# arkiven4/glow-tts

Hardware: AMD Instinct MI355X
Metric: mel_frames_per_sec_train_step (higher is better)
Workload: dtype bf16; 1 GPU; configs/base.json, LJSpeech-shaped synthetic batches, B=32/GPU, T_x<=150, T_y<=800, bf16 GEMMs; batch_per_gpu=32, T_x=150, T_y=800, batches_rotated=8, padded_frames_per_gpu_step=25600, rows_layout=ragged, graphs_captured=6, parallelism=dp1 (utterance-sharded, RCCL gradient all-reduce, fp32 on the wire), launch=one HIP graph per step (one per ragged-row bucket, captured up front)

## Files before the change

### glow-tts_amd/csrc/wn_boundary.hip

```cpp
#include "common.h"
#include "internal.h"
#include "mfma_frag.h"
#include "../../include/glowtts_hip.h"

namespace {

constexpr int H = 192, C = 160, HALF = 80, NL = 4, G = C / 4;
constexpr int BM = 64;
constexpr int AP = H + 8;
constexpr int XP = 136;
constexpr int ZP = C + 4;
constexpr int RD = 8;
#ifndef WNB_PHASES
#define WNB_PHASES 0
#endif
#if WNB_PHASES
__device__ unsigned long long g_wnb_ph[1024 * 48];
#define PH(i) do { if (threadIdx.x == 0 && blockIdx.x < 1024) g_wnb_ph[blockIdx.x * 48 + (i)] = __builtin_amdgcn_s_memtime(); } while (0)
#else
#define PH(i) do { } while (0)
#endif

template <int NB, int KK>
struct WRing { uint4 v[(KK < RD ? KK : RD)][NB]; };

template <int NB, int KK>
__device__ __forceinline__ void gemm_prefetch(const bf16_t* __restrict__ W, int KS, int nb0, int lane, WRing<NB, KK>& ring)
{
  constexpr int D = KK < RD ? KK : RD;
#pragma unroll
  for (int p = 0; p < D; ++p)
#pragma unroll
    for (int bn = 0; bn < NB; ++bn) ring.v[p][bn] = ldfrag(W, (nb0 + bn) * KS + p, lane);
}
template <int NB, int KK>
__device__ __forceinline__ void gemm_run(const bf16_t* __restrict__ W, int KS, int nb0, const bf16_t* Brow, int lane, WRing<NB, KK>& ring,
                                         f32x16_t (&acc)[NB])
{
  constexpr int D = KK < RD ? KK : RD, CH = 4;
#pragma unroll
  for (int k0 = 0; k0 < KK; k0 += CH) {
#pragma unroll
    for (int kk = k0; kk < k0 + CH && kk < KK; ++kk) {
      const bf16x8_t bfm = *reinterpret_cast<const bf16x8_t*>(Brow + kk * 16);
#pragma unroll
      for (int bn = 0; bn < NB; ++bn) acc[bn] = __builtin_amdgcn_mfma_f32_32x32x16_bf16(asfrag(ring.v[kk % D][bn]), bfm, acc[bn], 0, 0, 0);
    }
    if (k0 + D < KK) {
      __builtin_amdgcn_sched_barrier(0);
#pragma unroll
      for (int kk = k0; kk < k0 + CH && kk + D < KK; ++kk)
#pragma unroll
        for (int bn = 0; bn < NB; ++bn) ring.v[kk % D][bn] = ldfrag(W, (nb0 + bn) * KS + kk + D, lane);
      __builtin_amdgcn_sched_barrier(0);
    }
  }
}

__device__ __forceinline__ void utt_atomic_add(float* __restrict__ dst, float s, int utt, int lane)
{
#pragma unroll
  for (int off = 1; off < 64; off <<= 1) {
    const float v = __shfl_up(s, off);
    const int u = __shfl_up(utt, off);
    if (lane >= off && u == utt) s += v;
  }
  const int un = __shfl_down(utt, 1);
  if ((lane == 63 || un != utt) && s != 0.0f) atomicAdd(dst + utt, s);
}

template <int L>
__device__ __forceinline__ void skip_slice(const u32x4_t (&xr)[6], bf16_t* As, const bf16_t* __restrict__ Wskip, int wm, int wn, int r, int h,
                                           int lane, uint4 (&ring)[RD][3], f32x16_t (&acc)[3])
{
  constexpr int KK = NL * H / 16, kbase = L * (H / 16);
#pragma unroll
  for (int i = 0; i < 6; ++i) {
    const int chunk = threadIdx.x + 256 * i, row = chunk / 24, c8 = chunk - row * 24;
    *reinterpret_cast<u32x4_t*>(As + (L * BM + row) * AP + c8 * 8) = xr[i];
  }
  __syncthreads();
  const bf16_t* brow = As + (L * BM + 32 * wm + r) * AP + 8 * h;
  constexpr int CH = 4;
#pragma unroll
  for (int k0 = 0; k0 < H / 16; k0 += CH) {
#pragma unroll
    for (int k2 = k0; k2 < k0 + CH; ++k2) {
      const bf16x8_t bfm = *reinterpret_cast<const bf16x8_t*>(brow + k2 * 16);
#pragma unroll
      for (int bn = 0; bn < 3; ++bn) acc[bn] = __builtin_amdgcn_mfma_f32_32x32x16_bf16(asfrag(ring[(kbase + k2) % RD][bn]), bfm, acc[bn], 0, 0, 0);
    }
    if (kbase + k0 + RD < KK) {
      __builtin_amdgcn_sched_barrier(0);
#pragma unroll
      for (int k2 = k0; k2 < k0 + CH; ++k2)
#pragma unroll
        for (int bn = 0; bn < 3; ++bn)
          if (kbase + k2 + RD < KK) ring[(kbase + k2) % RD][bn] = ldfrag(Wskip, (3 * wn + bn) * KK + kbase + k2 + RD, lane);
      __builtin_amdgcn_sched_barrier(0);
    }
  }
}

__device__ __forceinline__ float4 sq_gather4(const float* __restrict__ y, int b, int t, int c, int T)
{
  const int p = c >= HALF, cc = c - HALF * p;
  const float* src = y + ((size_t)b * HALF + cc) * T + 2 * t + p;
  return make_float4(src[0], src[(size_t)T], src[2 * (size_t)T], src[3 * (size_t)T]);
}
__device__ __forceinline__ void sq_scatter4(float* __restrict__ y, int b, int t, int c, int T, const float4& v)
{
  const int p = c >= HALF, cc = c - HALF * p;
  float* dst = y + ((size_t)b * HALF + cc) * T + 2 * t + p;
  dst[0] = v.x; dst[(size_t)T] = v.y; dst[2 * (size_t)T] = v.z; dst[3 * (size_t)T] = v.w;
}

__device__ __forceinline__ void coop_store_rows(bf16_t* __restrict__ dst, int ld, const bf16_t* __restrict__ tile, int m0, int R)
{
  constexpr int CPR = H / 8;
#pragma unroll
  for (int i = 0; i < BM * CPR / 256; ++i) {
    const int idx = threadIdx.x + 256 * i, row = idx / CPR, c8 = idx - row * CPR, gm = m0 + row;
    if (gm < R) *reinterpret_cast<uint4*>(dst + (size_t)gm * ld + c8 * 8) = *reinterpret_cast<const uint4*>(tile + row * AP + c8 * 8);
  }
}

constexpr int PF_WGS = 64;
__device__ __forceinline__ void prefetch_images(const void* const (&ptr)[16], const uint32_t (&bytes)[16], int wg, uint32_t* sink)
{
  uint32_t acc = 0;
  const int gid = wg * 256 + threadIdx.x, nthr = PF_WGS * 256;
#pragma unroll
  for (int i = 0; i < 16; ++i) {
    if (!ptr[i]) break;
    const uint4* src = static_cast<const uint4*>(ptr[i]);
    const int n16 = (int)(bytes[i] >> 4);
    for (int c = gid; c < n16; c += 4 * nthr) {
      const uint4 v0 = src[c];
      const uint4 v1 = c + nthr < n16 ? src[c + nthr] : make_uint4(0, 0, 0, 0);
      const uint4 v2 = c + 2 * nthr < n16 ? src[c + 2 * nthr] : make_uint4(0, 0, 0, 0);
      const uint4 v3 = c + 3 * nthr < n16 ? src[c + 3 * nthr] : make_uint4(0, 0, 0, 0);
      acc ^= v0.x ^ v1.y ^ v2.z ^ v3.w;
    }
  }
  if (acc == 0x9E3779B9u && sink) *sink = acc;
}

constexpr int F_AS = 0;
constexpr int F_O = BM * AP * 2;
constexpr int F_Z = F_O + BM * ZP * 4;
constexpr int F_RS = (F_Z + BM * ZP * 4 > NL * BM * AP * 2 ? F_Z + BM * ZP * 4 : NL * BM * AP * 2);
constexpr int F_BIAS = F_RS + BM * 4;
constexpr int FWD_LDS = F_BIAS + 3 * H * 4 + BM * 4;
static_assert(F_O + BM * ZP * 4 <= 3 * BM * AP * 2, "the m | logs tile must stay clear of acts slice 3");

template <bool TAIL, bool HEAD>
__global__ __launch_bounds__(256) void gt_wn_boundary_fwd_kernel(gt_boundary_fwd_args a)
{
  extern __shared__ __attribute__((aligned(16))) unsigned char smem[];
  const int n_tiles = (a.R + BM - 1) / BM;
  if ((int)blockIdx.x >= n_tiles) { prefetch_images(a.pf_ptr, a.pf_bytes, blockIdx.x - n_tiles, reinterpret_cast<uint32_t*>(a.logdet)); return; }
  const int lane = threadIdx.x & 63, wave = threadIdx.x >> 6;
  const int r = lane & 31, h = lane >> 5, wm = wave >> 1, wn = wave & 1;
  const int m0 = blockIdx.x * BM, R = a.R;
  bf16_t* As = reinterpret_cast<bf16_t*>(smem + F_AS);
  float* Ot = reinterpret_cast<float*>(smem + F_O);
  float* Zt = reinterpret_cast<float*>(smem + F_Z);
  float* rowsum = reinterpret_cast<float*>(smem + F_RS);
  const int mrow = m0 + 32 * wm + r;
  const float rm_l = mrow < R ? a.rowmask[mrow] : 0.0f;
  float* Bs = reinterpret_cast<float*>(smem + F_BIAS);
  if (threadIdx.x < 3 * H / 4) {
    const int which = threadIdx.x / (H / 4), o = threadIdx.x - which * (H / 4);
    float4 v = make_float4(0.f, 0.f, 0.f, 0.f);
    if (which == 0) { if (TAIL) v = reinterpret_cast<const float4*>(a.b_skip)[o]; }
    else if (which == 1) { if (TAIL && o < C / 4) v = reinterpret_cast<const float4*>(a.b_end)[o]; }
    else if (HEAD) v = reinterpret_cast<const float4*>(a.b_start)[o];
    reinterpret_cast<float4*>(Bs)[threadIdx.x] = v;
  }
  float* Rm = Bs + 3 * H;
  if (threadIdx.x >= 192) {
    const int row = threadIdx.x - 192;
    Rm[row] = m0 + row < R ? a.rowmask[m0 + row] : 0.0f;
  }
  PH(0);

  if (TAIL) {
    const bf16_t* acts = static_cast<const bf16_t*>(a.acts);
    const bf16_t* Wskip = static_cast<const bf16_t*>(a.w_skip);
    u32x4_t xr[NL][6];
#pragma unroll
    for (int l = 0; l < NL; ++l)
#pragma unroll
      for (int i = 0; i < 6; ++i) {
        const int chunk = threadIdx.x + 256 * i, row = chunk / 24, c8 = chunk - row * 24;
        const int gm = m0 + row < R ? m0 + row : R - 1;
        xr[l][i] = *reinterpret_cast<const u32x4_t*>(acts + (size_t)gm * a.ldacts + l * H + c8 * 8);
      }
    if (threadIdx.x < BM) rowsum[threadIdx.x] = 0.0f;
    f32x16_t acc[3];
    acc_zero<3>(acc);
    constexpr int KK = NL * H / 16;
    uint4 ring[RD][3];
#pragma unroll
    for (int p = 0; p < RD; ++p)
#pragma unroll
      for (int bn = 0; bn < 3; ++bn) ring[p][bn] = ldfrag(Wskip, (3 * wn + bn) * KK + p, lane);
    PH(1);
    skip_slice<0>(xr[0], As, Wskip, wm, wn, r, h, lane, ring, acc);
    skip_slice<1>(xr[1], As, Wskip, wm, wn, r, h, lane, ring, acc);
    skip_slice<2>(xr[2], As, Wskip, wm, wn, r, h, lane, ring, acc);
    skip_slice<3>(xr[3], As, Wskip, wm, wn, r, h, lane, ring, acc);
    PH(2);
    WRing<3, H / 16> ring2;
    gemm_prefetch<3, H / 16>(static_cast<const bf16_t*>(a.w_end), a.ks_end, 3 * wn, lane, ring2);
    bf16_t* wn_out = static_cast<bf16_t*>(a.wn_out);
#pragma unroll
    for (int bn = 0; bn < 3; ++bn)
#pragma unroll
      for (int g = 0; g < 4; ++g) {
        const int n = 32 * (3 * wn + bn) + 8 * g + 4 * h;
        const float4 b4 = *reinterpret_cast<const float4*>(Bs + n);
        const uint2 v = pack4((acc[bn][4 * g] + b4.x) * rm_l, (acc[bn][4 * g + 1] + b4.y) * rm_l,
                              (acc[bn][4 * g + 2] + b4.z) * rm_l, (acc[bn][4 * g + 3] + b4.w) * rm_l);
        *reinterpret_cast<uint2*>(As + (32 * wm + r) * AP + n) = v;
      }
    __syncthreads();
    PH(3);
    coop_store_rows(wn_out, H, As, m0, R);
    float4 cy0[5], cy1[5];
    float crm[5];
#pragma unroll
    for (int k = 0; k < 5; ++k) {
      const int item = threadIdx.x + 256 * k, row = item / 20, c = 4 * (item - row * 20), gm = m0 + row < R ? m0 + row : R - 1;
      cy0[k] = *reinterpret_cast<const float4*>(a.y + (size_t)gm * C + c);
      cy1[k] = *reinterpret_cast<const float4*>(a.y + (size_t)gm * C + HALF + c);
      crm[k] = a.rowmask[gm];
    }
    f32x16_t acc2[3];
    acc_zero<3>(acc2);
    gemm_run<3, H / 16>(static_cast<const bf16_t*>(a.w_end), a.ks_end, 3 * wn, As + (32 * wm + r) * AP + 8 * h, lane, ring2, acc2);
    PH(4);
#pragma unroll
    for (int bn = 0; bn < 3; ++bn)
#pragma unroll
      for (int g = 0; g < 4; ++g) {
        const int n = 32 * (3 * wn + bn) + 8 * g + 4 * h;
        if (n < C) {
          const float4 b4 = *reinterpret_cast<const float4*>(Bs + H + n);
          *reinterpret_cast<float4*>(Ot + (32 * wm + r) * ZP + n) =
              make_float4(acc2[bn][4 * g] + b4.x, acc2[bn][4 * g + 1] + b4.y, acc2[bn][4 * g + 2] + b4.z, acc2[bn][4 * g + 3] + b4.w);
        }
      }
    __syncthreads();
    PH(5);
#pragma unroll
    for (int k = 0; k < 5; ++k) {
      const int item = threadIdx.x + 256 * k, row = item / 20, c = 4 * (item - row * 20), gm = m0 + row;
      float4 z0 = make_float4(0.f, 0.f, 0.f, 0.f), z1 = z0;
      if (gm < R) {
        const float rm = crm[k];
        const float4 mm = *reinterpret_cast<const float4*>(Ot + row * ZP + c);
        const float4 lr = *reinterpret_cast<const float4*>(Ot + row * ZP + HALF + c);
        z0 = cy0[k];
        const float4 y1 = cy1[k];
        float lg[4] = {lr.x, lr.y, lr.z, lr.w};
        if (a.sigmoid_scale) {
#pragma unroll
          for (int j = 0; j < 4; ++j) lg[j] = __logf(1e-6f + sigmoidf_(lg[j] + 2.0f));
        }
        z1 = make_float4((mm.x + __expf(lg[0]) * y1.x) * rm, (mm.y + __expf(lg[1]) * y1.y) * rm,
                         (mm.z + __expf(lg[2]) * y1.z) * rm, (mm.w + __expf(lg[3]) * y1.w) * rm);
        if (a.z) {
          *reinterpret_cast<float4*>(a.z + (size_t)gm * C + c) = z0;
          *reinterpret_cast<float4*>(a.z + (size_t)gm * C + HALF + c) = z1;
        }
        if (a.z_bct) {
          const int b = (int)a.rowbatch[gm], t = a.rowframe[gm];
          if (t >= 0 && t < a.len[b]) { sq_scatter4(a.z_bct, b, t, c, a.T, z0); sq_scatter4(a.z_bct, b, t, HALF + c, a.T, z1); }
        }
        *reinterpret_cast<float4*>(a.logs_raw + (size_t)gm * HALF + c) = lr;
        const float s = (lg[0] + lg[1] + lg[2] + lg[3]) * rm;
        if (s != 0.0f) atomicAdd(rowsum + row, s);
      }
      if (HEAD) {
        *reinterpret_cast<float4*>(Zt + row * ZP + c) = z0;
        *reinterpret_cast<float4*>(Zt + row * ZP + HALF + c) = z1;
      }
    }
    __syncthreads();
    PH(6);
    if (!HEAD && wave == 0) {
      const int gm = m0 + lane < R ? m0 + lane : R - 1;
      utt_atomic_add(a.logdet, rowsum[lane], a.rowutt[gm], lane);
    }
    PH(7);
  } else {
#pragma unroll
    for (int k = 0; k < 10; ++k) {
      const int item = threadIdx.x + 256 * k, row = item / 40, c = 4 * (item - row * 40), gm = m0 + row;
      float4 v = make_float4(0.f, 0.f, 0.f, 0.f);
      if (gm < R) {
        if (a.y_bct) {
          const int b = (int)a.rowbatch[gm], t = a.rowframe[gm];
          if (t >= 0 && t < a.len[b]) v = sq_gather4(a.y_bct, b, t, c, a.T);
          if (a.z) *reinterpret_cast<float4*>(a.z + (size_t)gm * C + c) = v;
        } else v = *reinterpret_cast<const float4*>(a.x_in + (size_t)gm * C + c);
      }
      *reinterpret_cast<float4*>(Zt + row * ZP + c) = v;
    }
    __syncthreads();
  }
  if (!HEAD) return;

  bf16_t* X0t = reinterpret_cast<bf16_t*>(smem + F_AS);
  WRing<3, HALF / 16> ring3;
  gemm_prefetch<3, HALF / 16>(static_cast<const bf16_t*>(a.w_start), a.ks_start, 3 * wn, lane, ring3);
  {
    float Wm[16];
#pragma unroll
    for (int i = 0; i < 16; ++i) Wm[i] = a.w_ic[i];
    bf16_t* y0b = static_cast<bf16_t*>(a.y0_bf16);
    constexpr int NPH = 256 / G;
    const int g = threadIdx.x % G, ph = threadIdx.x / G;
    if (ph < NPH) {
      const float e0 = __expf(a.an_logs[2 * g]), e1 = __expf(a.an_logs[2 * g + 1]);
      const float e2 = __expf(a.an_logs[HALF + 2 * g]), e3 = __expf(a.an_logs[HALF + 2 * g + 1]);
      const float c0 = a.an_bias[2 * g], c1 = a.an_bias[2 * g + 1], c2 = a.an_bias[HALF + 2 * g], c3 = a.an_bias[HALF + 2 * g + 1];
#pragma unroll
      for (int k = 0; k < (BM + NPH - 1) / NPH; ++k) {
        const int row = ph + NPH * k, gm = m0 + row;
        if (row < BM) {
          const float rm = Rm[row];
          const float2 xa = *reinterpret_cast<const float2*>(Zt + row * ZP + 2 * g);
          const float2 xb = *reinterpret_cast<const float2*>(Zt + row * ZP + HALF + 2 * g);
          const float a0 = c0 + e0 * xa.x, a1 = c1 + e1 * xa.y, a2 = c2 + e2 * xb.x, a3 = c3 + e3 * xb.y;
          float o[4];
#pragma unroll
          for (int q = 0; q < 4; ++q) o[q] = (Wm[q * 4] * a0 + Wm[q * 4 + 1] * a1 + Wm[q * 4 + 2] * a2 + Wm[q * 4 + 3] * a3) * rm;
          const uint32_t p01 = pack2bf(o[0], o[1]);
          if (gm < R) {
            *reinterpret_cast<float2*>(a.y_next + (size_t)gm * C + 2 * g) = make_float2(o[0], o[1]);
            *reinterpret_cast<float2*>(a.y_next + (size_t)gm * C + HALF + 2 * g) = make_float2(o[2], o[3]);
            *reinterpret_cast<uint32_t*>(y0b + (size_t)gm * HALF + 2 * g) = p01;
          }
          *reinterpret_cast<uint32_t*>(X0t + row * XP + 2 * g) = p01;
        }
      }
    }
  }
  __syncthreads();
  PH(8);
  {
    f32x16_t acc3[3];
    acc_zero<3>(acc3);
    gemm_run<3, HALF / 16>(static_cast<const bf16_t*>(a.w_start), a.ks_start, 3 * wn, X0t + (32 * wm + r) * XP + 8 * h, lane, ring3, acc3);
    PH(9);
    bf16_t* h0 = static_cast<bf16_t*>(a.h_next);
    bf16_t* Hst = reinterpret_cast<bf16_t*>(smem + F_O);
#pragma unroll
    for (int bn = 0; bn < 3; ++bn)
#pragma unroll
      for (int g = 0; g < 4; ++g) {
        const int n = 32 * (3 * wn + bn) + 8 * g + 4 * h;
        const float4 b4 = *reinterpret_cast<const float4*>(Bs + 2 * H + n);
        *reinterpret_cast<uint2*>(Hst + (32 * wm + r) * AP + n) =
            pack4((acc3[bn][4 * g] + b4.x) * rm_l, (acc3[bn][4 * g + 1] + b4.y) * rm_l,
                  (acc3[bn][4 * g + 2] + b4.z) * rm_l, (acc3[bn][4 * g + 3] + b4.w) * rm_l);
      }
    __syncthreads();
    PH(10);
    coop_store_rows(h0, H, Hst, m0, R);
  }
  if (TAIL && wave == 0) {
    const int gm = m0 + lane < R ? m0 + lane : R - 1;
    utt_atomic_add(a.logdet, rowsum[lane], a.rowutt[gm], lane);
  }
  if (blockIdx.x == 0) {
    const float per_frame = a.scal[0] + (float)G * a.scal[1];
    for (int b = threadIdx.x; b < a.B; b += 256) atomicAdd(a.logdet + b, per_frame * (float)a.len[b]);
  }
  PH(11);
}

constexpr int PG = 2 * C + 16;

__device__ __forceinline__ void param_grad_partials(const gt_boundary_bwd_args& a, const float* sL, const float* sB, const float* sW, float extra)
{
  float* row = a.pg_partial + (size_t)blockIdx.x * PG;
  for (int t = threadIdx.x; t < PG; t += 256) {
    if (t < 2 * C) {
      const int c = t < C ? t : t - C, hi = c >= HALF, cc = c - HALF * hi, g = cc >> 1, k = 2 * hi + (cc & 1);
      const float* sp = t < C ? sL : sB;
      float v = sp[g * 4 + k] + sp[(64 + g) * 4 + k] + sp[(128 + g) * 4 + k] + sp[(192 + g) * 4 + k];
      if (t < C) v += extra;
      row[t] = v;
    } else {
      const int i = t - 2 * C;
      row[t] = sW[i] + sW[16 + i] + sW[32 + i] + sW[48 + i] + (float)G * extra * a.scal[2 + i];
    }
  }
}

__device__ __forceinline__ void param_grad_atomics(const gt_boundary_bwd_args& a, const float* sL, const float* sB, const float* sW, int ph, int g)
{
  if (ph == 0 && g < G) {
    const int ch[4] = {2 * g, 2 * g + 1, HALF + 2 * g, HALF + 2 * g + 1};
#pragma unroll
    for (int k = 0; k < 4; ++k) {
      atomicAdd(a.d_an_logs + ch[k], sL[g * 4 + k] + sL[(64 + g) * 4 + k] + sL[(128 + g) * 4 + k] + sL[(192 + g) * 4 + k]);
      atomicAdd(a.d_an_bias + ch[k], sB[g * 4 + k] + sB[(64 + g) * 4 + k] + sB[(128 + g) * 4 + k] + sB[(192 + g) * 4 + k]);
    }
  }
  if (threadIdx.x < 16) atomicAdd(a.d_w_ic + threadIdx.x, sW[threadIdx.x] + sW[16 + threadIdx.x] + sW[32 + threadIdx.x] + sW[48 + threadIdx.x]);
}

constexpr int B_DH = 0;
constexpr int B_D = BM * AP * 2;
constexpr int B_DO = B_D + BM * ZP * 4;
constexpr int B_RED = B_DO + BM * AP * 2;
constexpr int BWD_LDS = B_RED + 2 * 4 * 64 * 4 * 4 + 4 * 16 * 4 + 16;

template <bool HEADB, bool TAILB>
__global__ __launch_bounds__(256) void gt_wn_boundary_bwd_kernel(gt_boundary_bwd_args a)
{
  extern __shared__ __attribute__((aligned(16))) unsigned char smem[];
  const int n_tiles = (a.R + BM - 1) / BM;
  if ((int)blockIdx.x >= n_tiles) { prefetch_images(a.pf_ptr, a.pf_bytes, blockIdx.x - n_tiles, nullptr); return; }
  const int lane = threadIdx.x & 63, wave = threadIdx.x >> 6;
  const int r = lane & 31, h = lane >> 5, wm = wave >> 1, wn = wave & 1;
  const int m0 = blockIdx.x * BM, R = a.R;
  bf16_t* Dh = reinterpret_cast<bf16_t*>(smem + B_DH);
  float* Dt = reinterpret_cast<float*>(smem + B_D);
  bf16_t* Dout = reinterpret_cast<bf16_t*>(smem + B_DO);
  const int mrow = m0 + 32 * wm + r;
  const float rm_l = mrow < R ? a.rowmask[mrow] : 0.0f;
  PH(0);

  if (HEADB) {
    const bf16_t* dh = static_cast<const bf16_t*>(a.dh);
#pragma unroll
    for (int i = 0; i < 6; ++i) {
      const int chunk = threadIdx.x + 256 * i, row = chunk / 24, c8 = chunk - row * 24;
      const int gm = m0 + row < R ? m0 + row : R - 1;
      *reinterpret_cast<uint4*>(Dh + row * AP + c8 * 8) = *reinterpret_cast<const uint4*>(dh + (size_t)gm * H + c8 * 8);
    }
    WRing<2, H / 16> ring1;
    gemm_prefetch<2, H / 16>(static_cast<const bf16_t*>(a.w_start_d), a.ks_start_d, 2 * wn, lane, ring1);
    __syncthreads();
    PH(1);
    f32x16_t acc[2];
    acc_zero<2>(acc);
    gemm_run<2, H / 16>(static_cast<const bf16_t*>(a.w_start_d), a.ks_start_d, 2 * wn, Dh + (32 * wm + r) * AP + 8 * h, lane, ring1, acc);
#pragma unroll
    for (int bn = 0; bn < 2; ++bn)
#pragma unroll
      for (int g = 0; g < 4; ++g) {
        const int n = 32 * (2 * wn + bn) + 8 * g + 4 * h;
        if (n < HALF)
          *reinterpret_cast<float4*>(Dt + (32 * wm + r) * ZP + n) = make_float4(acc[bn][4 * g], acc[bn][4 * g + 1], acc[bn][4 * g + 2], acc[bn][4 * g + 3]);
      }
    __syncthreads();
    PH(2);
    float* sL = reinterpret_cast<float*>(smem + B_RED);
    float* sB = sL + 4 * 64 * 4;
    float* sW = sB + 4 * 64 * 4;
    float* sred = sW + 4 * 16;
    float extra = 0.f;
    if (blockIdx.x == 0) {
      float sv = 0.f;
      for (int b = threadIdx.x; b < a.B; b += 256) sv += a.dlogdet[b] * (float)a.len[b];
      sv = wave_sum(sv);
      if (lane == 0) sred[wave] = sv;
      __syncthreads();
      sv = sred[0] + sred[1] + sred[2] + sred[3];
      if (a.pg_partial) extra = sv;
      else {
        for (int c = threadIdx.x; c < C; c += 256) atomicAdd(a.d_an_logs + c, sv);
        if (threadIdx.x < 16) atomicAdd(a.d_w_ic + threadIdx.x, (float)G * sv * a.scal[2 + threadIdx.x]);
      }
    }
    const int g = lane, ph = wave;
    float accW[16], accL[4] = {0, 0, 0, 0}, accB[4] = {0, 0, 0, 0};
#pragma unroll
    for (int i = 0; i < 16; ++i) accW[i] = 0.f;
    if (g < G) {
      const int ch[4] = {2 * g, 2 * g + 1, HALF + 2 * g, HALF + 2 * g + 1};
      float el[4], bs[4], Wm[16];
#pragma unroll
      for (int k = 0; k < 4; ++k) { el[k] = __expf(a.an_logs[ch[k]]); bs[k] = a.an_bias[ch[k]]; }
#pragma unroll
      for (int i = 0; i < 16; ++i) Wm[i] = a.w_ic[i];
      const float* __restrict__ xp = a.x;
      const float* __restrict__ dip = a.dx_in;
#pragma unroll
      for (int rb = 0; rb < BM / 4; rb += 8) {
        float2 xa[8], xb[8], da[8], db[8];
        float rmv[8];
#pragma unroll
        for (int u = 0; u < 8; ++u) {
          const int row = ph + 4 * (rb + u), gm = m0 + row < R ? m0 + row : R - 1;
          xa[u] = *reinterpret_cast<const float2*>(xp + (size_t)gm * C + 2 * g);
          xb[u] = *reinterpret_cast<const float2*>(xp + (size_t)gm * C + HALF + 2 * g);
          da[u] = *reinterpret_cast<const float2*>(dip + (size_t)gm * C + 2 * g);
          db[u] = *reinterpret_cast<const float2*>(dip + (size_t)gm * C + HALF + 2 * g);
          rmv[u] = m0 + row < R ? a.rowmask[gm] : 0.0f;
        }
#pragma unroll
        for (int u = 0; u < 8; ++u) {
          const int row = ph + 4 * (rb + u), gm = m0 + row;
          const float rm = rmv[u];
          const float2 ds = *reinterpret_cast<const float2*>(Dt + row * ZP + 2 * g);
          const float xv[4] = {xa[u].x, xa[u].y, xb[u].x, xb[u].y};
          const float dym[4] = {(da[u].x + ds.x) * rm, (da[u].y + ds.y) * rm, db[u].x * rm, db[u].y * rm};
          float av[4], d_a[4], dxv[4];
#pragma unroll
          for (int k = 0; k < 4; ++k) av[k] = bs[k] + el[k] * xv[k];
#pragma unroll
          for (int i = 0; i < 4; ++i) d_a[i] = Wm[i] * dym[0] + Wm[4 + i] * dym[1] + Wm[8 + i] * dym[2] + Wm[12 + i] * dym[3];
#pragma unroll
          for (int o = 0; o < 4; ++o)
#pragma unroll
            for (int i = 0; i < 4; ++i) accW[o * 4 + i] += dym[o] * av[i];
#pragma unroll
          for (int k = 0; k < 4; ++k) { accB[k] += d_a[k]; accL[k] += d_a[k] * xv[k] * el[k]; dxv[k] = d_a[k] * el[k]; }
          if (TAILB) {
            *reinterpret_cast<float2*>(Dt + row * ZP + 2 * g) = make_float2(dxv[0], dxv[1]);
            *reinterpret_cast<float2*>(Dt + row * ZP + HALF + 2 * g) = make_float2(dxv[2], dxv[3]);
          } else if (gm < R) {
            if (a.dx_bct) {
              const int b = (int)a.rowbatch[gm], t = a.rowframe[gm];
              if (t >= 0 && t < a.len[b]) {
                float* d0 = a.dx_bct + ((size_t)b * HALF + 2 * g) * a.T + 2 * t;
                d0[0] = dxv[0]; d0[(size_t)a.T] = dxv[1]; d0[1] = dxv[2]; d0[(size_t)a.T + 1] = dxv[3];
              }
            } else {
              *reinterpret_cast<float2*>(a.dx_out + (size_t)gm * C + 2 * g) = make_float2(dxv[0], dxv[1]);
              *reinterpret_cast<float2*>(a.dx_out + (size_t)gm * C + HALF + 2 * g) = make_float2(dxv[2], dxv[3]);
            }
          }
        }
      }
    }
    PH(3);
#pragma unroll
    for (int k = 0; k < 4; ++k) { sL[(ph * 64 + g) * 4 + k] = accL[k]; sB[(ph * 64 + g) * 4 + k] = accB[k]; }
#pragma unroll
    for (int i = 0; i < 16; ++i) accW[i] = wave_sum(accW[i]);
    if (g == 0) {
#pragma unroll
      for (int i = 0; i < 16; ++i) sW[ph * 16 + i] = accW[i];
    }
    __syncthreads();
    PH(4);
    if (a.pg_partial) param_grad_partials(a, sL, sB, sW, extra);
    if (!TAILB) {
      if (!a.pg_partial) param_grad_atomics(a, sL, sB, sW, wave, lane);
      return;
    }
  } else {
#pragma unroll
    for (int k = 0; k < 10; ++k) {
      const int item = threadIdx.x + 256 * k, row = item / 40, c = 4 * (item - row * 40), gm = m0 + row;
      float4 v = make_float4(0.f, 0.f, 0.f, 0.f);
      if (gm < R) {
        if (a.dz_bct) {
          const int b = (int)a.rowbatch[gm], t = a.rowframe[gm];
          if (t >= 0 && t < a.len[b]) v = sq_gather4(a.dz_bct, b, t, c, a.T);
        } else v = *reinterpret_cast<const float4*>(a.dz_in + (size_t)gm * C + c);
      }
      *reinterpret_cast<float4*>(Dt + row * ZP + c) = v;
    }
    __syncthreads();
  }

  bf16_t* dout = static_cast<bf16_t*>(a.dout);
  WRing<3, C / 16> ring2;
  gemm_prefetch<3, C / 16>(static_cast<const bf16_t*>(a.w_end_d), a.ks_end_d, 3 * wn, lane, ring2);
  {
    float4 lr4[5], y14[5];
    float rmv[5], dldv[5];
#pragma unroll
    for (int k = 0; k < 5; ++k) {
      const int item = threadIdx.x + 256 * k, row = item / 20, c = 4 * (item - row * 20), gm = m0 + row < R ? m0 + row : R - 1;
      lr4[k] = *reinterpret_cast<const float4*>(a.logs_raw + (size_t)gm * HALF + c);
      y14[k] = *reinterpret_cast<const float4*>(a.y + (size_t)gm * C + HALF + c);
      rmv[k] = a.rowmask[gm];
      dldv[k] = a.dlogdet[a.rowutt[gm]];
    }
#pragma unroll
    for (int k = 0; k < 5; ++k) {
      const int item = threadIdx.x + 256 * k, row = item / 20, c = 4 * (item - row * 20), gm = m0 + row;
      uint2 pm = make_uint2(0, 0), pl = make_uint2(0, 0);
      if (gm < R) {
        const float rm = rmv[k];
        const float4 dz0 = *reinterpret_cast<const float4*>(Dt + row * ZP + c);
        const float4 dz1r = *reinterpret_cast<const float4*>(Dt + row * ZP + HALF + c);
        const float dld = dldv[k] * rm;
        const float dz1[4] = {dz1r.x * rm, dz1r.y * rm, dz1r.z * rm, dz1r.w * rm};
        const float lraw[4] = {lr4[k].x, lr4[k].y, lr4[k].z, lr4[k].w}, y1v[4] = {y14[k].x, y14[k].y, y14[k].z, y14[k].w};
        float dx1[4], dlg[4];
#pragma unroll
        for (int j = 0; j < 4; ++j) {
          float lg = lraw[j], dl_draw = 1.0f;
          if (a.sigmoid_scale) { const float sg = sigmoidf_(lraw[j] + 2.0f); lg = __logf(1e-6f + sg); dl_draw = sg * (1.0f - sg) / (1e-6f + sg); }
          const float e = __expf(lg);
          dx1[j] = dz1[j] * e;
          dlg[j] = (dz1[j] * e * y1v[j] + dld) * dl_draw;
        }
        *reinterpret_cast<float4*>(a.dx_out + (size_t)gm * C + c) = dz0;
        *reinterpret_cast<float4*>(a.dx_out + (size_t)gm * C + HALF + c) = make_float4(dx1[0], dx1[1], dx1[2], dx1[3]);
        pm = pack4(dz1[0], dz1[1], dz1[2], dz1[3]);
        pl = pack4(dlg[0], dlg[1], dlg[2], dlg[3]);
        *reinterpret_cast<uint2*>(dout + (size_t)gm * C + c) = pm;
        *reinterpret_cast<uint2*>(dout + (size_t)gm * C + HALF + c) = pl;
      }
      *reinterpret_cast<uint2*>(Dout + row * AP + c) = pm;
      *reinterpret_cast<uint2*>(Dout + row * AP + HALF + c) = pl;
    }
  }
  __syncthreads();
  PH(5);
  bf16_t* At = Dh;
  const bf16_t* Wsd = static_cast<const bf16_t*>(a.w_skip_d);
  constexpr int KS2 = H / 16, NS = NL * KS2;
  uint4 ring3[RD][3];
  {
    f32x16_t acc[3];
    acc_zero<3>(acc);
    gemm_run<3, C / 16>(static_cast<const bf16_t*>(a.w_end_d), a.ks_end_d, 3 * wn, Dout + (32 * wm + r) * AP + 8 * h, lane, ring2, acc);
    PH(6);
#pragma unroll
    for (int p = 0; p < RD; ++p)
#pragma unroll
      for (int bn = 0; bn < 3; ++bn) ring3[p][bn] = ldfrag(Wsd, (6 * (p / KS2) + 3 * wn + bn) * a.ks_skip_d + p % KS2, lane);
#pragma unroll
    for (int bn = 0; bn < 3; ++bn)
#pragma unroll
      for (int g = 0; g < 4; ++g) {
        const int n = 32 * (3 * wn + bn) + 8 * g + 4 * h;
        const uint2 v = pack4(acc[bn][4 * g] * rm_l, acc[bn][4 * g + 1] * rm_l, acc[bn][4 * g + 2] * rm_l, acc[bn][4 * g + 3] * rm_l);
        *reinterpret_cast<uint2*>(At + (32 * wm + r) * AP + n) = v;
      }
  }
  __syncthreads();
  PH(7);
  coop_store_rows(static_cast<bf16_t*>(a.dwn_out), H, At, m0, R);
  PH(8);
  bf16_t* via = static_cast<bf16_t*>(a.via_skip);
  const bf16_t* brow = At + (32 * wm + r) * AP + 8 * h;
#pragma unroll
  for (int l = 0; l < NL; ++l) {
    f32x16_t acc[3];
    acc_zero<3>(acc);
#pragma unroll
    for (int k0 = 0; k0 < KS2; k0 += 4) {
#pragma unroll
      for (int kk = k0; kk < k0 + 4; ++kk) {
        const int st = l * KS2 + kk;
        const bf16x8_t bfm = *reinterpret_cast<const bf16x8_t*>(brow + kk * 16);
#pragma unroll
        for (int bn = 0; bn < 3; ++bn) acc[bn] = __builtin_amdgcn_mfma_f32_32x32x16_bf16(asfrag(ring3[st % RD][bn]), bfm, acc[bn], 0, 0, 0);
      }
      if (l * KS2 + k0 + RD < NS) {
        __builtin_amdgcn_sched_barrier(0);
#pragma unroll
        for (int kk = k0; kk < k0 + 4; ++kk) {
          const int st = l * KS2 + kk, nx = st + RD;
#pragma unroll
          for (int bn = 0; bn < 3; ++bn)
            if (nx < NS) ring3[st % RD][bn] = ldfrag(Wsd, (6 * (nx / KS2) + 3 * wn + bn) * a.ks_skip_d + nx % KS2, lane);
        }
        __builtin_amdgcn_sched_barrier(0);
      }
    }
    bf16_t* Vst = reinterpret_cast<bf16_t*>(smem + ((l & 1) ? B_DO : B_D));
#pragma unroll
    for (int bn = 0; bn < 3; ++bn)
#pragma unroll
      for (int g = 0; g < 4; ++g) {
        const int n = 32 * (3 * wn + bn) + 8 * g + 4 * h;
        *reinterpret_cast<uint2*>(Vst + (32 * wm + r) * AP + n) = pack4(acc[bn][4 * g], acc[bn][4 * g + 1], acc[bn][4 * g + 2], acc[bn][4 * g + 3]);
      }
    __syncthreads();
    coop_store_rows(via + l * H, a.ldvs, Vst, m0, R);
    PH(9 + l);
  }
  if (HEADB && !a.pg_partial) {
    const float* sL = reinterpret_cast<const float*>(smem + B_RED);
    param_grad_atomics(a, sL, sL + 4 * 64 * 4, sL + 2 * 4 * 64 * 4, wave, lane);
  }
}

__global__ __launch_bounds__(384) void gt_boundary_param_reduce_kernel(const float* __restrict__ pg, int n_wg, float* const* __restrict__ dst)
{
  const int b = blockIdx.x, t = threadIdx.x;
  if (t >= PG) return;
  const int per = (n_wg + gridDim.y - 1) / gridDim.y, w0 = blockIdx.y * per, w1 = min(n_wg, w0 + per);
  const float* p = pg + (size_t)b * n_wg * PG + t;
  float s0 = 0.f, s1 = 0.f, s2 = 0.f, s3 = 0.f;
  int w = w0;
  for (; w + 4 <= w1; w += 4) { s0 += p[(size_t)w * PG]; s1 += p[(size_t)(w + 1) * PG]; s2 += p[(size_t)(w + 2) * PG]; s3 += p[(size_t)(w + 3) * PG]; }
  for (; w < w1; ++w) s0 += p[(size_t)w * PG];
  float* d = t < C ? dst[3 * b] + t : (t < 2 * C ? dst[3 * b + 1] + (t - C) : dst[3 * b + 2] + (t - 2 * C));
  atomicAdd(d, (s0 + s1) + (s2 + s3));
}

constexpr int REV_LDS = FWD_LDS;

template <bool TAIL, bool HEAD>
__global__ __launch_bounds__(256) void gt_wn_boundary_rev_kernel(gt_boundary_rev_args a)
{
  extern __shared__ __attribute__((aligned(16))) unsigned char smem[];
  const int n_tiles = (a.R + BM - 1) / BM;
  if ((int)blockIdx.x >= n_tiles) { prefetch_images(a.pf_ptr, a.pf_bytes, blockIdx.x - n_tiles, nullptr); return; }
  const int lane = threadIdx.x & 63, wave = threadIdx.x >> 6;
  const int r = lane & 31, h = lane >> 5, wm = wave >> 1, wn = wave & 1;
  const int m0 = blockIdx.x * BM, R = a.R;
  bf16_t* As = reinterpret_cast<bf16_t*>(smem + F_AS);
  float* Ot = reinterpret_cast<float*>(smem + F_O);
  float* Zt = reinterpret_cast<float*>(smem + F_Z);
  bf16_t* X0t = reinterpret_cast<bf16_t*>(smem + F_AS);
  const int mrow = m0 + 32 * wm + r;
  const float rm_l = mrow < R ? a.rowmask[mrow] : 0.0f;
  float* Bs = reinterpret_cast<float*>(smem + F_BIAS);
  if (threadIdx.x < 3 * H / 4) {
    const int which = threadIdx.x / (H / 4), o = threadIdx.x - which * (H / 4);
    float4 v = make_float4(0.f, 0.f, 0.f, 0.f);
    if (which == 0) { if (TAIL) v = reinterpret_cast<const float4*>(a.b_skip)[o]; }
    else if (which == 1) { if (TAIL && o < C / 4) v = reinterpret_cast<const float4*>(a.b_end)[o]; }
    else if (HEAD) v = reinterpret_cast<const float4*>(a.b_start)[o];
    reinterpret_cast<float4*>(Bs)[threadIdx.x] = v;
  }
  float* Rm = Bs + 3 * H;
  if (threadIdx.x >= 192) {
    const int row = threadIdx.x - 192;
    Rm[row] = m0 + row < R ? a.rowmask[m0 + row] : 0.0f;
  }
  WRing<3, HALF / 16> ring3;

  if (TAIL) {
    const bf16_t* acts = static_cast<const bf16_t*>(a.acts);
    const bf16_t* Wskip = static_cast<const bf16_t*>(a.w_skip);
    u32x4_t xr[NL][6];
#pragma unroll
    for (int l = 0; l < NL; ++l)
#pragma unroll
      for (int i = 0; i < 6; ++i) {
        const int chunk = threadIdx.x + 256 * i, row = chunk / 24, c8 = chunk - row * 24;
        const int gm = m0 + row < R ? m0 + row : R - 1;
        xr[l][i] = *reinterpret_cast<const u32x4_t*>(acts + (size_t)gm * a.ldacts + l * H + c8 * 8);
      }
    f32x16_t acc[3];
    acc_zero<3>(acc);
    constexpr int KK = NL * H / 16;
    uint4 ring[RD][3];
#pragma unroll
    for (int p = 0; p < RD; ++p)
#pragma unroll
      for (int bn = 0; bn < 3; ++bn) ring[p][bn] = ldfrag(Wskip, (3 * wn + bn) * KK + p, lane);
    skip_slice<0>(xr[0], As, Wskip, wm, wn, r, h, lane, ring, acc);
    skip_slice<1>(xr[1], As, Wskip, wm, wn, r, h, lane, ring, acc);
    skip_slice<2>(xr[2], As, Wskip, wm, wn, r, h, lane, ring, acc);
    skip_slice<3>(xr[3], As, Wskip, wm, wn, r, h, lane, ring, acc);
    WRing<3, H / 16> ring2;
    gemm_prefetch<3, H / 16>(static_cast<const bf16_t*>(a.w_end), a.ks_end, 3 * wn, lane, ring2);
#pragma unroll
    for (int bn = 0; bn < 3; ++bn)
#pragma unroll
      for (int g = 0; g < 4; ++g) {
        const int n = 32 * (3 * wn + bn) + 8 * g + 4 * h;
        const float4 b4 = *reinterpret_cast<const float4*>(Bs + n);
        *reinterpret_cast<uint2*>(As + (32 * wm + r) * AP + n) =
            pack4((acc[bn][4 * g] + b4.x) * rm_l, (acc[bn][4 * g + 1] + b4.y) * rm_l,
                  (acc[bn][4 * g + 2] + b4.z) * rm_l, (acc[bn][4 * g + 3] + b4.w) * rm_l);
      }
    __syncthreads();
    auto z_load = [&](int k, int half) {
      const int item = threadIdx.x + 256 * k, row = item / 20, c = 4 * (item - row * 20), gm = m0 + row < R ? m0 + row : R - 1;
      return *reinterpret_cast<const float4*>(a.z + (size_t)gm * C + half * HALF + c);
    };
    const float4 za0 = z_load(0, 0), za1 = z_load(1, 0), za2 = z_load(2, 0), za3 = z_load(3, 0), za4 = z_load(4, 0);
    const float4 zb0 = z_load(0, 1), zb1 = z_load(1, 1), zb2 = z_load(2, 1), zb3 = z_load(3, 1), zb4 = z_load(4, 1);
    f32x16_t acc2[3];
    acc_zero<3>(acc2);
    gemm_run<3, H / 16>(static_cast<const bf16_t*>(a.w_end), a.ks_end, 3 * wn, As + (32 * wm + r) * AP + 8 * h, lane, ring2, acc2);
    if (HEAD) gemm_prefetch<3, HALF / 16>(static_cast<const bf16_t*>(a.w_start), a.ks_start, 3 * wn, lane, ring3);
    auto z_put = [&](int k, const float4& v0, const float4& v1) {
      const int item = threadIdx.x + 256 * k, row = item / 20, c = 4 * (item - row * 20);
      *reinterpret_cast<float4*>(Zt + row * ZP + c) = v0;
      *reinterpret_cast<float4*>(Zt + row * ZP + HALF + c) = v1;
    };
    z_put(0, za0, zb0); z_put(1, za1, zb1); z_put(2, za2, zb2); z_put(3, za3, zb3); z_put(4, za4, zb4);
#pragma unroll
    for (int bn = 0; bn < 3; ++bn)
#pragma unroll
      for (int g = 0; g < 4; ++g) {
        const int n = 32 * (3 * wn + bn) + 8 * g + 4 * h;
        if (n < C) {
          const float4 b4 = *reinterpret_cast<const float4*>(Bs + H + n);
          *reinterpret_cast<float4*>(Ot + (32 * wm + r) * ZP + n) =
              make_float4(acc2[bn][4 * g] + b4.x, acc2[bn][4 * g + 1] + b4.y, acc2[bn][4 * g + 2] + b4.z, acc2[bn][4 * g + 3] + b4.w);
        }
      }
    __syncthreads();
#pragma unroll
    for (int k = 0; k < 5; ++k) {
      const int item = threadIdx.x + 256 * k, row = item / 20, c = 4 * (item - row * 20);
      const float rm = Rm[row];
      const float4 mm = *reinterpret_cast<const float4*>(Ot + row * ZP + c);
      const float4 lr = *reinterpret_cast<const float4*>(Ot + row * ZP + HALF + c);
      float lg[4] = {lr.x, lr.y, lr.z, lr.w};
      if (a.sigmoid_scale) {
#pragma unroll
        for (int j = 0; j < 4; ++j) lg[j] = __logf(1e-6f + sigmoidf_(lg[j] + 2.0f));
      }
      const float4 z1 = *reinterpret_cast<const float4*>(Zt + row * ZP + HALF + c);
      *reinterpret_cast<float4*>(Zt + row * ZP + HALF + c) =
          make_float4((z1.x - mm.x) * __expf(-lg[0]) * rm, (z1.y - mm.y) * __expf(-lg[1]) * rm,
                      (z1.z - mm.z) * __expf(-lg[2]) * rm, (z1.w - mm.w) * __expf(-lg[3]) * rm);
    }
    __syncthreads();
    {
      constexpr int NPH = 256 / G;
      const int g = threadIdx.x % G, ph = threadIdx.x / G;
      if (ph < NPH) {
        float Wi[16];
#pragma unroll
        for (int i = 0; i < 16; ++i) Wi[i] = a.scal[2 + i];
        const float e0 = __expf(-a.an_logs[2 * g]), e1 = __expf(-a.an_logs[2 * g + 1]);
        const float e2 = __expf(-a.an_logs[HALF + 2 * g]), e3 = __expf(-a.an_logs[HALF + 2 * g + 1]);
        const float c0 = a.an_bias[2 * g], c1 = a.an_bias[2 * g + 1], c2 = a.an_bias[HALF + 2 * g], c3 = a.an_bias[HALF + 2 * g + 1];
#pragma unroll
        for (int k = 0; k < (BM + NPH - 1) / NPH; ++k) {
          const int row = ph + NPH * k, gm = m0 + row;
          if (row < BM) {
            const float rm = Rm[row];
            const float2 ua = *reinterpret_cast<const float2*>(Zt + row * ZP + 2 * g);
            const float2 ub = *reinterpret_cast<const float2*>(Zt + row * ZP + HALF + 2 * g);
            float o[4];
#pragma unroll
            for (int q = 0; q < 4; ++q) o[q] = (Wi[q] * ua.x + Wi[4 + q] * ua.y + Wi[8 + q] * ub.x + Wi[12 + q] * ub.y) * rm;
            o[0] = (o[0] - c0) * e0 * rm; o[1] = (o[1] - c1) * e1 * rm; o[2] = (o[2] - c2) * e2 * rm; o[3] = (o[3] - c3) * e3 * rm;
            if (gm < R) {
              if (a.x) {
                *reinterpret_cast<float2*>(a.x + (size_t)gm * C + 2 * g) = make_float2(o[0], o[1]);
                *reinterpret_cast<float2*>(a.x + (size_t)gm * C + HALF + 2 * g) = make_float2(o[2], o[3]);
              }
              if (!HEAD && a.x_bct) {
                const int b = (int)a.rowbatch[gm], t = a.rowframe[gm];
                if (t >= 0 && t < a.len[b]) {
                  float* d0 = a.x_bct + ((size_t)b * HALF + 2 * g) * a.T + 2 * t;
                  d0[0] = o[0]; d0[(size_t)a.T] = o[1]; d0[1] = o[2]; d0[(size_t)a.T + 1] = o[3];
                }
              }
            }
            if (HEAD) *reinterpret_cast<uint32_t*>(X0t + row * XP + 2 * g) = pack2bf(o[0], o[1]);
          }
        }
      }
    }
  } else {
    gemm_prefetch<3, HALF / 16>(static_cast<const bf16_t*>(a.w_start), a.ks_start, 3 * wn, lane, ring3);
#pragma unroll
    for (int k = 0; k < 10; ++k) {
      const int item = threadIdx.x + 256 * k, row = item / 40, c = 4 * (item - row * 40), gm = m0 + row;
      float4 v = make_float4(0.f, 0.f, 0.f, 0.f);
      if (gm < R) {
        if (a.z_bct) {
          const int b = (int)a.rowbatch[gm], t = a.rowframe[gm];
          if (t >= 0 && t < a.len[b]) v = sq_gather4(a.z_bct, b, t, c, a.T);
          *reinterpret_cast<float4*>(a.x + (size_t)gm * C + c) = v;
        } else v = *reinterpret_cast<const float4*>(a.x_in + (size_t)gm * C + c);
      }
      if (c < HALF) *reinterpret_cast<uint2*>(X0t + row * XP + c) = pack4(v.x, v.y, v.z, v.w);
    }
  }
  if (!HEAD) return;
  __syncthreads();
  {
    f32x16_t acc3[3];
    acc_zero<3>(acc3);
    gemm_run<3, HALF / 16>(static_cast<const bf16_t*>(a.w_start), a.ks_start, 3 * wn, X0t + (32 * wm + r) * XP + 8 * h, lane, ring3, acc3);
    bf16_t* Hst = reinterpret_cast<bf16_t*>(smem + F_O);
#pragma unroll
    for (int bn = 0; bn < 3; ++bn)
#pragma unroll
      for (int g = 0; g < 4; ++g) {
        const int n = 32 * (3 * wn + bn) + 8 * g + 4 * h;
        const float4 b4 = *reinterpret_cast<const float4*>(Bs + 2 * H + n);
        *reinterpret_cast<uint2*>(Hst + (32 * wm + r) * AP + n) =
            pack4((acc3[bn][4 * g] + b4.x) * rm_l, (acc3[bn][4 * g + 1] + b4.y) * rm_l,
                  (acc3[bn][4 * g + 2] + b4.z) * rm_l, (acc3[bn][4 * g + 3] + b4.w) * rm_l);
      }
    __syncthreads();
    coop_store_rows(static_cast<bf16_t*>(a.h_next), H, Hst, m0, R);
  }
}

template <typename K>
int opt_in_lds(K kernel, int bytes)
{
  return hipFuncSetAttribute(reinterpret_cast<const void*>(kernel), hipFuncAttributeMaxDynamicSharedMemorySize, bytes) == hipSuccess ? 0 : -1;
}

}

#if WNB_PHASES
extern "C" int gt_dev_wnb_phases(void* dst, size_t bytes)
{
  return hipMemcpyFromSymbol(dst, HIP_SYMBOL(g_wnb_ph), bytes < sizeof(g_wnb_ph) ? bytes : sizeof(g_wnb_ph)) == hipSuccess ? 0 : -1;
}
#endif

extern "C" int gt_wn_boundary_fwd(const gt_boundary_fwd_args* args, void* stream)
{
  if (!args) return GT_E_INVAL;
  const gt_boundary_fwd_args& a = *args;
  if (a.R < 0) return GT_E_INVAL;
  if (a.R == 0) return GT_OK;
  if (a.H != H || a.C != C || a.n_layers != NL) return GT_E_UNSUPPORTED;
  const bool tail = a.acts != nullptr, head = a.y_next != nullptr;
  if (!tail && !head) return GT_E_INVAL;
  if (!a.rowmask) return GT_E_INVAL;
  if (tail) {
    if (!a.w_skip || !a.b_skip || !a.w_end || !a.b_end || !a.y || !a.wn_out || !a.logs_raw || (!a.z && !a.z_bct) || !a.logdet || !a.rowutt) return GT_E_INVAL;
    if (a.z_bct && (head || !a.rowbatch || !a.rowframe || !a.len || a.T <= 0)) return GT_E_INVAL;
    if (a.ldacts < NL * H || (a.ldacts & 7) || a.ks_end < H / 16) return GT_E_INVAL;
    if (!al16(a.acts) || !al16(a.w_skip) || !al16(a.w_end) || !al16(a.b_skip) || !al16(a.b_end) || !al16(a.y) || !al16(a.wn_out) ||
        !al16(a.logs_raw) || !al16(a.z)) return GT_E_ALIGN;
  } else if (a.y_bct ? (!a.rowbatch || !a.rowframe || a.T <= 0) : (!a.x_in || !al16(a.x_in))) return GT_E_INVAL;
  if (head) {
    if (!a.an_logs || !a.an_bias || !a.w_ic || !a.scal || !a.len || a.B <= 0 || !a.logdet || !a.y0_bf16 || !a.w_start || !a.b_start || !a.h_next)
      return GT_E_INVAL;
    if (a.ks_start < HALF / 16) return GT_E_INVAL;
    if (!al16(a.y_next) || !al16(a.y0_bf16) || !al16(a.w_start) || !al16(a.b_start) || !al16(a.h_next)) return GT_E_ALIGN;
  }
  static bool attr = false;
  if (!attr) {
    if (opt_in_lds(&gt_wn_boundary_fwd_kernel<true, true>, FWD_LDS) || opt_in_lds(&gt_wn_boundary_fwd_kernel<true, false>, FWD_LDS) ||
        opt_in_lds(&gt_wn_boundary_fwd_kernel<false, true>, FWD_LDS)) return GT_E_LAUNCH;
    attr = true;
  }
  for (int i = 0; i < 16; ++i) if (a.pf_ptr[i] && (!al16(a.pf_ptr[i]) || (a.pf_bytes[i] & 15))) return GT_E_ALIGN;
  const dim3 grid((a.R + BM - 1) / BM + (a.pf_ptr[0] ? PF_WGS : 0)), block(256);
  hipStream_t st = static_cast<hipStream_t>(stream);
  if (tail && head) hipLaunchKernelGGL((gt_wn_boundary_fwd_kernel<true, true>), grid, block, FWD_LDS, st, a);
  else if (tail)    hipLaunchKernelGGL((gt_wn_boundary_fwd_kernel<true, false>), grid, block, FWD_LDS, st, a);
  else              hipLaunchKernelGGL((gt_wn_boundary_fwd_kernel<false, true>), grid, block, FWD_LDS, st, a);
  return gt_launch_status(__func__);
}

extern "C" int gt_boundary_rev_args_size(void) { return (int)sizeof(gt_boundary_rev_args); }

extern "C" int gt_wn_boundary_rev(const gt_boundary_rev_args* args, void* stream)
{
  if (!args) return GT_E_INVAL;
  const gt_boundary_rev_args& a = *args;
  if (a.R < 0) return GT_E_INVAL;
  if (a.R == 0) return GT_OK;
  if (a.H != H || a.C != C || a.n_layers != NL) return GT_E_INVAL;
  const bool tail = a.acts != nullptr, head = a.h_next != nullptr;
  if (!tail && !head) return GT_E_INVAL;
  if (!a.rowmask) return GT_E_INVAL;
  if ((a.z_bct || a.x_bct) && (!a.rowbatch || !a.rowframe || !a.len || a.T <= 0 || (a.T & 1))) return GT_E_INVAL;
  if (tail) {
    if (!a.w_skip || !a.b_skip || !a.w_end || !a.b_end || !a.z || !a.an_logs || !a.an_bias || !a.scal || (!a.x && !a.x_bct)) return GT_E_INVAL;
    if (a.x_bct && head) return GT_E_INVAL;
    if (head && !a.x) return GT_E_INVAL;
    if (a.ldacts < NL * H || (a.ldacts & 7) || a.ks_end < H / 16) return GT_E_INVAL;
    if (!al16(a.acts) || !al16(a.w_skip) || !al16(a.w_end) || !al16(a.b_skip) || !al16(a.b_end) || !al16(a.z) || !al16(a.x)) return GT_E_ALIGN;
  } else {
    if (a.z_bct ? !a.x : !a.x_in) return GT_E_INVAL;
    if (!al16(a.x_in) || !al16(a.x)) return GT_E_ALIGN;
  }
  if (head) {
    if (!a.w_start || !a.b_start || a.ks_start < HALF / 16) return GT_E_INVAL;
    if (!al16(a.w_start) || !al16(a.b_start) || !al16(a.h_next)) return GT_E_ALIGN;
  }
  for (int i = 0; i < 16; ++i) if (a.pf_ptr[i] && (!al16(a.pf_ptr[i]) || (a.pf_bytes[i] & 15))) return GT_E_ALIGN;
  static bool attr = false;
  if (!attr) {
    if (opt_in_lds(&gt_wn_boundary_rev_kernel<true, true>, REV_LDS) || opt_in_lds(&gt_wn_boundary_rev_kernel<true, false>, REV_LDS) ||
        opt_in_lds(&gt_wn_boundary_rev_kernel<false, true>, REV_LDS)) return GT_E_LAUNCH;
    attr = true;
  }
  const dim3 grid((a.R + BM - 1) / BM + (a.pf_ptr[0] ? PF_WGS : 0)), block(256);
  hipStream_t st = static_cast<hipStream_t>(stream);
  if (tail && head) hipLaunchKernelGGL((gt_wn_boundary_rev_kernel<true, true>), grid, block, REV_LDS, st, a);
  else if (tail)    hipLaunchKernelGGL((gt_wn_boundary_rev_kernel<true, false>), grid, block, REV_LDS, st, a);
  else              hipLaunchKernelGGL((gt_wn_boundary_rev_kernel<false, true>), grid, block, REV_LDS, st, a);
  return gt_launch_status(__func__);
}

extern "C" int gt_boundary_param_partials(void) { return PG; }

extern "C" int gt_boundary_param_reduce(const float* partials, int n_wg, int n_blocks, float* const* dst, void* stream)
{
  if (!partials || !dst || n_wg <= 0 || n_blocks < 0) return GT_E_INVAL;
  if (n_blocks == 0) return GT_OK;
  hipLaunchKernelGGL(gt_boundary_param_reduce_kernel, dim3(n_blocks, 8), dim3(384), 0, static_cast<hipStream_t>(stream), partials, n_wg, dst);
  return gt_launch_status(__func__);
}

extern "C" int gt_wn_boundary_bwd(const gt_boundary_bwd_args* args, void* stream)
{
  if (!args) return GT_E_INVAL;
  const gt_boundary_bwd_args& a = *args;
  if (a.R < 0) return GT_E_INVAL;
  if (a.R == 0) return GT_OK;
  if (a.H != H || a.C != C || a.n_layers != NL) return GT_E_UNSUPPORTED;
  const bool headb = a.dh != nullptr, tailb = a.dout != nullptr;
  if (!headb && !tailb) return GT_E_INVAL;
  if (!a.rowmask || (!a.dx_out && !a.dx_bct) || !al16(a.dx_out)) return GT_E_INVAL;
  if ((a.dx_bct || a.dz_bct) && (!a.rowbatch || !a.rowframe || !a.len || a.T <= 0)) return GT_E_INVAL;
  if (a.dx_bct && tailb) return GT_E_INVAL;
  if (headb) {
    if (!a.w_start_d || !a.dx_in || !a.x || !a.an_logs || !a.an_bias || !a.w_ic || !a.scal || !a.len || !a.dlogdet || a.B <= 0 ||
        !a.d_an_logs || !a.d_an_bias || !a.d_w_ic) return GT_E_INVAL;
    if (a.ks_start_d < H / 16) return GT_E_INVAL;
    if (!al16(a.dh) || !al16(a.w_start_d) || !al16(a.dx_in) || !al16(a.x)) return GT_E_ALIGN;
  } else if (!a.dz_bct && (!a.dz_in || !al16(a.dz_in))) return GT_E_INVAL;
  if (tailb) {
    if (!a.logs_raw || !a.y || !a.dlogdet || !a.rowutt || !a.w_end_d || !a.dwn_out || !a.w_skip_d || !a.via_skip) return GT_E_INVAL;
    if (a.ks_end_d < C / 16 || a.ks_skip_d < H / 16 || a.ldvs < NL * H || (a.ldvs & 7)) return GT_E_INVAL;
    if (!al16(a.logs_raw) || !al16(a.y) || !al16(a.dout) || !al16(a.w_end_d) || !al16(a.dwn_out) || !al16(a.w_skip_d) || !al16(a.via_skip))
      return GT_E_ALIGN;
  }
  static bool attr = false;
  if (!attr) {
    if (opt_in_lds(&gt_wn_boundary_bwd_kernel<true, true>, BWD_LDS) || opt_in_lds(&gt_wn_boundary_bwd_kernel<true, false>, BWD_LDS) ||
        opt_in_lds(&gt_wn_boundary_bwd_kernel<false, true>, BWD_LDS)) return GT_E_LAUNCH;
    attr = true;
  }
  for (int i = 0; i < 16; ++i) if (a.pf_ptr[i] && (!al16(a.pf_ptr[i]) || (a.pf_bytes[i] & 15))) return GT_E_ALIGN;
  const dim3 grid((a.R + BM - 1) / BM + (a.pf_ptr[0] ? PF_WGS : 0)), block(256);
  hipStream_t st = static_cast<hipStream_t>(stream);
  if (headb && tailb) hipLaunchKernelGGL((gt_wn_boundary_bwd_kernel<true, true>), grid, block, BWD_LDS, st, a);
  else if (headb)     hipLaunchKernelGGL((gt_wn_boundary_bwd_kernel<true, false>), grid, block, BWD_LDS, st, a);
  else                hipLaunchKernelGGL((gt_wn_boundary_bwd_kernel<false, true>), grid, block, BWD_LDS, st, a);
  return gt_launch_status(__func__);
}
```

Baseline: 4.501 million mel-frames/s.

## Split WaveNet boundary kernels across eight waves with uneven N-block assignment

The forward and backward WaveNet boundary kernels now launch with 512 threads instead of 256. Waves 0-3 compute two 32-column output blocks and waves 4-7 compute the remaining one, so all six N-blocks of each 64-row tile are still covered. Cooperative load and store loops, the reduction slices and the LDS sizing are rescaled to the new thread count, with an 8-way fold for the parameter-gradient partials. The aim is more waves in flight per tile to hide latency in the MFMA and weight-fragment loads. The cost is an uneven per-wave load and different register and LDS pressure per workgroup.

```diff
diff --git a/glow-tts_amd/csrc/wn_boundary.hip b/glow-tts_amd/csrc/wn_boundary.hip
--- a/glow-tts_amd/csrc/wn_boundary.hip
+++ b/glow-tts_amd/csrc/wn_boundary.hip
@@ -15,8 +15,9 @@
 #define WNB_PHASES 0
 #endif
 #if WNB_PHASES
-__device__ unsigned long long g_wnb_ph[1024 * 48];
-#define PH(i) do { if (threadIdx.x == 0 && blockIdx.x < 1024) g_wnb_ph[blockIdx.x * 48 + (i)] = __builtin_amdgcn_s_memtime(); } while (0)
+__device__ unsigned long long g_wnb_ph[2 * 1024 * 48];
+#define PH(i) do { if ((threadIdx.x == 0 || threadIdx.x == 256) && blockIdx.x < 1024)                                                \
+                     g_wnb_ph[((threadIdx.x >> 8) * 1024 + blockIdx.x) * 48 + (i)] = __builtin_amdgcn_s_memtime(); } while (0)
 #else
 #define PH(i) do { } while (0)
 #endif
@@ -69,14 +70,14 @@
   if ((lane == 63 || un != utt) && s != 0.0f) atomicAdd(dst + utt, s);
 }
 
-template <int L>
-__device__ __forceinline__ void skip_slice(const u32x4_t (&xr)[6], bf16_t* As, const bf16_t* __restrict__ Wskip, int wm, int wn, int r, int h,
-                                           int lane, uint4 (&ring)[RD][3], f32x16_t (&acc)[3])
+template <int L, int NB, int NT>
+__device__ __forceinline__ void skip_slice(const u32x4_t (&xr)[BM * 24 / NT], bf16_t* As, const bf16_t* __restrict__ Wskip, int wm, int nb0, int r, int h,
+                                           int lane, uint4 (&ring)[RD][NB], f32x16_t (&acc)[NB])
 {
   constexpr int KK = NL * H / 16, kbase = L * (H / 16);
 #pragma unroll
-  for (int i = 0; i < 6; ++i) {
-    const int chunk = threadIdx.x + 256 * i, row = chunk / 24, c8 = chunk - row * 24;
+  for (int i = 0; i < BM * 24 / NT; ++i) {
+    const int chunk = threadIdx.x + NT * i, row = chunk / 24, c8 = chunk - row * 24;
     *reinterpret_cast<u32x4_t*>(As + (L * BM + row) * AP + c8 * 8) = xr[i];
   }
   __syncthreads();
@@ -88,15 +89,15 @@
     for (int k2 = k0; k2 < k0 + CH; ++k2) {
       const bf16x8_t bfm = *reinterpret_cast<const bf16x8_t*>(brow + k2 * 16);
 #pragma unroll
-      for (int bn = 0; bn < 3; ++bn) acc[bn] = __builtin_amdgcn_mfma_f32_32x32x16_bf16(asfrag(ring[(kbase + k2) % RD][bn]), bfm, acc[bn], 0, 0, 0);
+      for (int bn = 0; bn < NB; ++bn) acc[bn] = __builtin_amdgcn_mfma_f32_32x32x16_bf16(asfrag(ring[(kbase + k2) % RD][bn]), bfm, acc[bn], 0, 0, 0);
     }
     if (kbase + k0 + RD < KK) {
       __builtin_amdgcn_sched_barrier(0);
 #pragma unroll
       for (int k2 = k0; k2 < k0 + CH; ++k2)
 #pragma unroll
-        for (int bn = 0; bn < 3; ++bn)
-          if (kbase + k2 + RD < KK) ring[(kbase + k2) % RD][bn] = ldfrag(Wskip, (3 * wn + bn) * KK + kbase + k2 + RD, lane);
+        for (int bn = 0; bn < NB; ++bn)
+          if (kbase + k2 + RD < KK) ring[(kbase + k2) % RD][bn] = ldfrag(Wskip, (nb0 + bn) * KK + kbase + k2 + RD, lane);
       __builtin_amdgcn_sched_barrier(0);
     }
   }
@@ -115,21 +116,23 @@
   dst[0] = v.x; dst[(size_t)T] = v.y; dst[2 * (size_t)T] = v.z; dst[3 * (size_t)T] = v.w;
 }
 
+template <int NT>
 __device__ __forceinline__ void coop_store_rows(bf16_t* __restrict__ dst, int ld, const bf16_t* __restrict__ tile, int m0, int R)
 {
   constexpr int CPR = H / 8;
 #pragma unroll
-  for (int i = 0; i < BM * CPR / 256; ++i) {
-    const int idx = threadIdx.x + 256 * i, row = idx / CPR, c8 = idx - row * CPR, gm = m0 + row;
+  for (int i = 0; i < BM * CPR / NT; ++i) {
+    const int idx = threadIdx.x + NT * i, row = idx / CPR, c8 = idx - row * CPR, gm = m0 + row;
     if (gm < R) *reinterpret_cast<uint4*>(dst + (size_t)gm * ld + c8 * 8) = *reinterpret_cast<const uint4*>(tile + row * AP + c8 * 8);
   }
 }
 
 constexpr int PF_WGS = 64;
+template <int NT>
 __device__ __forceinline__ void prefetch_images(const void* const (&ptr)[16], const uint32_t (&bytes)[16], int wg, uint32_t* sink)
 {
   uint32_t acc = 0;
-  const int gid = wg * 256 + threadIdx.x, nthr = PF_WGS * 256;
+  const int gid = wg * NT + threadIdx.x, nthr = PF_WGS * NT;
 #pragma unroll
   for (int i = 0; i < 16; ++i) {
     if (!ptr[i]) break;
@@ -154,14 +157,17 @@
 constexpr int FWD_LDS = F_BIAS + 3 * H * 4 + BM * 4;
 static_assert(F_O + BM * ZP * 4 <= 3 * BM * AP * 2, "the m | logs tile must stay clear of acts slice 3");
 
-template <bool TAIL, bool HEAD>
-__global__ __launch_bounds__(256) void gt_wn_boundary_fwd_kernel(gt_boundary_fwd_args a)
-{
-  extern __shared__ __attribute__((aligned(16))) unsigned char smem[];
-  const int n_tiles = (a.R + BM - 1) / BM;
-  if ((int)blockIdx.x >= n_tiles) { prefetch_images(a.pf_ptr, a.pf_bytes, blockIdx.x - n_tiles, reinterpret_cast<uint32_t*>(a.logdet)); return; }
+constexpr int NT2 = 512;
+#define WAVES_2 __attribute__((amdgpu_waves_per_eu(2, 2)))
+__device__ __forceinline__ int wave_scalar() { return __builtin_amdgcn_readfirstlane((int)(threadIdx.x >> 6)); }
+
+template <bool TAIL, bool HEAD, int NB>
+__device__ __forceinline__ void boundary_fwd_wave(const gt_boundary_fwd_args& a, unsigned char* smem)
+{
+  constexpr int NT = NT2;
   const int lane = threadIdx.x & 63, wave = threadIdx.x >> 6;
-  const int r = lane & 31, h = lane >> 5, wm = wave >> 1, wn = wave & 1;
+  const int r = lane & 31, h = lane >> 5, wm = (wave & 3) >> 1, wn = wave & 1;
+  const int nb0 = 3 * wn + (NB == 2 ? 0 : 2);
   const int m0 = blockIdx.x * BM, R = a.R;
   bf16_t* As = reinterpret_cast<bf16_t*>(smem + F_AS);
   float* Ot = reinterpret_cast<float*>(smem + F_O);
@@ -179,8 +185,8 @@
     reinterpret_cast<float4*>(Bs)[threadIdx.x] = v;
   }
   float* Rm = Bs + 3 * H;
-  if (threadIdx.x >= 192) {
-    const int row = threadIdx.x - 192;
+  if (threadIdx.x >= NT - BM) {
+    const int row = threadIdx.x - (NT - BM);
     Rm[row] = m0 + row < R ? a.rowmask[m0 + row] : 0.0f;
   }
   PH(0);
@@ -188,38 +194,39 @@
   if (TAIL) {
     const bf16_t* acts = static_cast<const bf16_t*>(a.acts);
     const bf16_t* Wskip = static_cast<const bf16_t*>(a.w_skip);
-    u32x4_t xr[NL][6];
+    constexpr int NCH = BM * 24 / NT;
+    u32x4_t xr[NL][NCH];
 #pragma unroll
     for (int l = 0; l < NL; ++l)
 #pragma unroll
-      for (int i = 0; i < 6; ++i) {
-        const int chunk = threadIdx.x + 256 * i, row = chunk / 24, c8 = chunk - row * 24;
+      for (int i = 0; i < NCH; ++i) {
+        const int chunk = threadIdx.x + NT * i, row = chunk / 24, c8 = chunk - row * 24;
         const int gm = m0 + row < R ? m0 + row : R - 1;
         xr[l][i] = *reinterpret_cast<const u32x4_t*>(acts + (size_t)gm * a.ldacts + l * H + c8 * 8);
       }
     if (threadIdx.x < BM) rowsum[threadIdx.x] = 0.0f;
-    f32x16_t acc[3];
-    acc_zero<3>(acc);
+    f32x16_t acc[NB];
+    acc_zero<NB>(acc);
     constexpr int KK = NL * H / 16;
-    uint4 ring[RD][3];
+    uint4 ring[RD][NB];
 #pragma unroll
     for (int p = 0; p < RD; ++p)
 #pragma unroll
-      for (int bn = 0; bn < 3; ++bn) ring[p][bn] = ldfrag(Wskip, (3 * wn + bn) * KK + p, lane);
+      for (int bn = 0; bn < NB; ++bn) ring[p][bn] = ldfrag(Wskip, (nb0 + bn) * KK + p, lane);
     PH(1);
-    skip_slice<0>(xr[0], As, Wskip, wm, wn, r, h, lane, ring, acc);
-    skip_slice<1>(xr[1], As, Wskip, wm, wn, r, h, lane, ring, acc);
-    skip_slice<2>(xr[2], As, Wskip, wm, wn, r, h, lane, ring, acc);
-    skip_slice<3>(xr[3], As, Wskip, wm, wn, r, h, lane, ring, acc);
+    skip_slice<0, NB, NT>(xr[0], As, Wskip, wm, nb0, r, h, lane, ring, acc);
+    skip_slice<1, NB, NT>(xr[1], As, Wskip, wm, nb0, r, h, lane, ring, acc);
+    skip_slice<2, NB, NT>(xr[2], As, Wskip, wm, nb0, r, h, lane, ring, acc);
+    skip_slice<3, NB, NT>(xr[3], As, Wskip, wm, nb0, r, h, lane, ring, acc);
     PH(2);
-    WRing<3, H / 16> ring2;
-    gemm_prefetch<3, H / 16>(static_cast<const bf16_t*>(a.w_end), a.ks_end, 3 * wn, lane, ring2);
+    WRing<NB, H / 16> ring2;
+    gemm_prefetch<NB, H / 16>(static_cast<const bf16_t*>(a.w_end), a.ks_end, nb0, lane, ring2);
     bf16_t* wn_out = static_cast<bf16_t*>(a.wn_out);
 #pragma unroll
-    for (int bn = 0; bn < 3; ++bn)
+    for (int bn = 0; bn < NB; ++bn)
 #pragma unroll
       for (int g = 0; g < 4; ++g) {
-        const int n = 32 * (3 * wn + bn) + 8 * g + 4 * h;
+        const int n = 32 * (nb0 + bn) + 8 * g + 4 * h;
         const float4 b4 = *reinterpret_cast<const float4*>(Bs + n);
         const uint2 v = pack4((acc[bn][4 * g] + b4.x) * rm_l, (acc[bn][4 * g + 1] + b4.y) * rm_l,
                               (acc[bn][4 * g + 2] + b4.z) * rm_l, (acc[bn][4 * g + 3] + b4.w) * rm_l);
@@ -227,25 +234,28 @@
       }
     __syncthreads();
     PH(3);
-    coop_store_rows(wn_out, H, As, m0, R);
-    float4 cy0[5], cy1[5];
-    float crm[5];
-#pragma unroll
-    for (int k = 0; k < 5; ++k) {
-      const int item = threadIdx.x + 256 * k, row = item / 20, c = 4 * (item - row * 20), gm = m0 + row < R ? m0 + row : R - 1;
-      cy0[k] = *reinterpret_cast<const float4*>(a.y + (size_t)gm * C + c);
-      cy1[k] = *reinterpret_cast<const float4*>(a.y + (size_t)gm * C + HALF + c);
-      crm[k] = a.rowmask[gm];
-    }
-    f32x16_t acc2[3];
-    acc_zero<3>(acc2);
-    gemm_run<3, H / 16>(static_cast<const bf16_t*>(a.w_end), a.ks_end, 3 * wn, As + (32 * wm + r) * AP + 8 * h, lane, ring2, acc2);
+    coop_store_rows<NT>(wn_out, H, As, m0, R);
+    constexpr int NCI = (BM * 20 + NT - 1) / NT;
+    float4 cy0[NCI], cy1[NCI];
+    float crm[NCI];
+#pragma unroll
+    for (int k = 0; k < NCI; ++k) {
+      const int item = threadIdx.x + NT * k, row = item / 20, c = 4 * (item - row * 20), gm = m0 + row < R ? m0 + row : R - 1;
+      if (item < BM * 20) {
+        cy0[k] = *reinterpret_cast<const float4*>(a.y + (size_t)gm * C + c);
+        cy1[k] = *reinterpret_cast<const float4*>(a.y + (size_t)gm * C + HALF + c);
+        crm[k] = a.rowmask[gm];
+      }
+    }
+    f32x16_t acc2[NB];
+    acc_zero<NB>(acc2);
+    gemm_run<NB, H / 16>(static_cast<const bf16_t*>(a.w_end), a.ks_end, nb0, As + (32 * wm + r) * AP + 8 * h, lane, ring2, acc2);
     PH(4);
 #pragma unroll
-    for (int bn = 0; bn < 3; ++bn)
+    for (int bn = 0; bn < NB; ++bn)
 #pragma unroll
       for (int g = 0; g < 4; ++g) {
-        const int n = 32 * (3 * wn + bn) + 8 * g + 4 * h;
+        const int n = 32 * (nb0 + bn) + 8 * g + 4 * h;
         if (n < C) {
           const float4 b4 = *reinterpret_cast<const float4*>(Bs + H + n);
           *reinterpret_cast<float4*>(Ot + (32 * wm + r) * ZP + n) =
@@ -255,8 +265,9 @@
     __syncthreads();
     PH(5);
 #pragma unroll
-    for (int k = 0; k < 5; ++k) {
-      const int item = threadIdx.x + 256 * k, row = item / 20, c = 4 * (item - row * 20), gm = m0 + row;
+    for (int k = 0; k < NCI; ++k) {
+      const int item = threadIdx.x + NT * k, row = item / 20, c = 4 * (item - row * 20), gm = m0 + row;
+      if (item >= BM * 20) break;
       float4 z0 = make_float4(0.f, 0.f, 0.f, 0.f), z1 = z0;
       if (gm < R) {
         const float rm = crm[k];
@@ -297,8 +308,8 @@
     PH(7);
   } else {
 #pragma unroll
-    for (int k = 0; k < 10; ++k) {
-      const int item = threadIdx.x + 256 * k, row = item / 40, c = 4 * (item - row * 40), gm = m0 + row;
+    for (int k = 0; k < BM * 40 / NT; ++k) {
+      const int item = threadIdx.x + NT * k, row = item / 40, c = 4 * (item - row * 40), gm = m0 + row;
       float4 v = make_float4(0.f, 0.f, 0.f, 0.f);
       if (gm < R) {
         if (a.y_bct) {
@@ -314,14 +325,14 @@
   if (!HEAD) return;
 
   bf16_t* X0t = reinterpret_cast<bf16_t*>(smem + F_AS);
-  WRing<3, HALF / 16> ring3;
-  gemm_prefetch<3, HALF / 16>(static_cast<const bf16_t*>(a.w_start), a.ks_start, 3 * wn, lane, ring3);
+  WRing<NB, HALF / 16> ring3;
+  gemm_prefetch<NB, HALF / 16>(static_cast<const bf16_t*>(a.w_start), a.ks_start, nb0, lane, ring3);
   {
     float Wm[16];
 #pragma unroll
     for (int i = 0; i < 16; ++i) Wm[i] = a.w_ic[i];
     bf16_t* y0b = static_cast<bf16_t*>(a.y0_bf16);
-    constexpr int NPH = 256 / G;
+    constexpr int NPH = NT / G;
     const int g = threadIdx.x % G, ph = threadIdx.x / G;
     if (ph < NPH) {
       const float e0 = __expf(a.an_logs[2 * g]), e1 = __expf(a.an_logs[2 * g + 1]);
@@ -352,17 +363,17 @@
   __syncthreads();
   PH(8);
   {
-    f32x16_t acc3[3];
-    acc_zero<3>(acc3);
-    gemm_run<3, HALF / 16>(static_cast<const bf16_t*>(a.w_start), a.ks_start, 3 * wn, X0t + (32 * wm + r) * XP + 8 * h, lane, ring3, acc3);
+    f32x16_t acc3[NB];
+    acc_zero<NB>(acc3);
+    gemm_run<NB, HALF / 16>(static_cast<const bf16_t*>(a.w_start), a.ks_start, nb0, X0t + (32 * wm + r) * XP + 8 * h, lane, ring3, acc3);
     PH(9);
     bf16_t* h0 = static_cast<bf16_t*>(a.h_next);
     bf16_t* Hst = reinterpret_cast<bf16_t*>(smem + F_O);
 #pragma unroll
-    for (int bn = 0; bn < 3; ++bn)
+    for (int bn = 0; bn < NB; ++bn)
 #pragma unroll
       for (int g = 0; g < 4; ++g) {
-        const int n = 32 * (3 * wn + bn) + 8 * g + 4 * h;
+        const int n = 32 * (nb0 + bn) + 8 * g + 4 * h;
         const float4 b4 = *reinterpret_cast<const float4*>(Bs + 2 * H + n);
         *reinterpret_cast<uint2*>(Hst + (32 * wm + r) * AP + n) =
             pack4((acc3[bn][4 * g] + b4.x) * rm_l, (acc3[bn][4 * g + 1] + b4.y) * rm_l,
@@ -370,7 +381,7 @@
       }
     __syncthreads();
     PH(10);
-    coop_store_rows(h0, H, Hst, m0, R);
+    coop_store_rows<NT>(h0, H, Hst, m0, R);
   }
   if (TAIL && wave == 0) {
     const int gm = m0 + lane < R ? m0 + lane : R - 1;
@@ -378,26 +389,42 @@
   }
   if (blockIdx.x == 0) {
     const float per_frame = a.scal[0] + (float)G * a.scal[1];
-    for (int b = threadIdx.x; b < a.B; b += 256) atomicAdd(a.logdet + b, per_frame * (float)a.len[b]);
+    for (int b = threadIdx.x; b < a.B; b += NT) atomicAdd(a.logdet + b, per_frame * (float)a.len[b]);
   }
   PH(11);
 }
 
+template <bool TAIL, bool HEAD>
+__global__ __launch_bounds__(NT2) WAVES_2 void gt_wn_boundary_fwd_kernel(gt_boundary_fwd_args a)
+{
+  extern __shared__ __attribute__((aligned(16))) unsigned char smem[];
+  const int n_tiles = (a.R + BM - 1) / BM;
+  if ((int)blockIdx.x >= n_tiles) { prefetch_images<NT2>(a.pf_ptr, a.pf_bytes, blockIdx.x - n_tiles, reinterpret_cast<uint32_t*>(a.logdet)); return; }
+  if (wave_scalar() < 4) boundary_fwd_wave<TAIL, HEAD, 2>(a, smem);
+  else boundary_fwd_wave<TAIL, HEAD, 1>(a, smem);
+}
+
 constexpr int PG = 2 * C + 16;
 
+constexpr int NSL = NT2 / 64;
+__device__ __forceinline__ float fold8(const float* sp, int stride)
+{
+  return (((sp[0] + sp[4 * stride]) + (sp[stride] + sp[5 * stride])) + (sp[2 * stride] + sp[6 * stride])) + (sp[3 * stride] + sp[7 * stride]);
+}
+
 __device__ __forceinline__ void param_grad_partials(const gt_boundary_bwd_args& a, const float* sL, const float* sB, const float* sW, float extra)
 {
   float* row = a.pg_partial + (size_t)blockIdx.x * PG;
-  for (int t = threadIdx.x; t < PG; t += 256) {
+  for (int t = threadIdx.x; t < PG; t += NT2) {
     if (t < 2 * C) {
       const int c = t < C ? t : t - C, hi = c >= HALF, cc = c - HALF * hi, g = cc >> 1, k = 2 * hi + (cc & 1);
       const float* sp = t < C ? sL : sB;
-      float v = sp[g * 4 + k] + sp[(64 + g) * 4 + k] + sp[(128 + g) * 4 + k] + sp[(192 + g) * 4 + k];
+      float v = fold8(sp + g * 4 + k, 64 * 4);
       if (t < C) v += extra;
       row[t] = v;
     } else {
       const int i = t - 2 * C;
-      row[t] = sW[i] + sW[16 + i] + sW[32 + i] + sW[48 + i] + (float)G * extra * a.scal[2 + i];
+      row[t] = fold8(sW + i, 16) + (float)G * extra * a.scal[2 + i];
     }
   }
 }
@@ -408,27 +435,27 @@
     const int ch[4] = {2 * g, 2 * g + 1, HALF + 2 * g, HALF + 2 * g + 1};
 #pragma unroll
     for (int k = 0; k < 4; ++k) {
-      atomicAdd(a.d_an_logs + ch[k], sL[g * 4 + k] + sL[(64 + g) * 4 + k] + sL[(128 + g) * 4 + k] + sL[(192 + g) * 4 + k]);
-      atomicAdd(a.d_an_bias + ch[k], sB[g * 4 + k] + sB[(64 + g) * 4 + k] + sB[(128 + g) * 4 + k] + sB[(192 + g) * 4 + k]);
-    }
-  }
-  if (threadIdx.x < 16) atomicAdd(a.d_w_ic + threadIdx.x, sW[threadIdx.x] + sW[16 + threadIdx.x] + sW[32 + threadIdx.x] + sW[48 + threadIdx.x]);
+      atomicAdd(a.d_an_logs + ch[k], fold8(sL + g * 4 + k, 64 * 4));
+      atomicAdd(a.d_an_bias + ch[k], fold8(sB + g * 4 + k, 64 * 4));
+    }
+  }
+  if (threadIdx.x < 16) atomicAdd(a.d_w_ic + threadIdx.x, fold8(sW + threadIdx.x, 16));
 }
 
 constexpr int B_DH = 0;
 constexpr int B_D = BM * AP * 2;
 constexpr int B_DO = B_D + BM * ZP * 4;
 constexpr int B_RED = B_DO + BM * AP * 2;
-constexpr int BWD_LDS = B_RED + 2 * 4 * 64 * 4 * 4 + 4 * 16 * 4 + 16;
-
-template <bool HEADB, bool TAILB>
-__global__ __launch_bounds__(256) void gt_wn_boundary_bwd_kernel(gt_boundary_bwd_args a)
-{
-  extern __shared__ __attribute__((aligned(16))) unsigned char smem[];
-  const int n_tiles = (a.R + BM - 1) / BM;
-  if ((int)blockIdx.x >= n_tiles) { prefetch_images(a.pf_ptr, a.pf_bytes, blockIdx.x - n_tiles, nullptr); return; }
+constexpr int BWD_LDS = B_RED + 2 * NSL * 64 * 4 * 4 + NSL * 16 * 4 + NSL * 4;
+static_assert(BWD_LDS <= 160 * 1024, "one workgroup's LDS");
+
+template <bool HEADB, bool TAILB, int NB>
+__device__ __forceinline__ void boundary_bwd_wave(const gt_boundary_bwd_args& a, unsigned char* smem)
+{
+  constexpr int NT = NT2;
   const int lane = threadIdx.x & 63, wave = threadIdx.x >> 6;
-  const int r = lane & 31, h = lane >> 5, wm = wave >> 1, wn = wave & 1;
+  const int r = lane & 31, h = lane >> 5, wm = (wave & 3) >> 1, wn = wave & 1;
+  const int nb0 = 3 * wn + (NB == 2 ? 0 : 2);
   const int m0 = blockIdx.x * BM, R = a.R;
   bf16_t* Dh = reinterpret_cast<bf16_t*>(smem + B_DH);
   float* Dt = reinterpret_cast<float*>(smem + B_D);
@@ -439,48 +466,47 @@
 
   if (HEADB) {
     const bf16_t* dh = static_cast<const bf16_t*>(a.dh);
-#pragma unroll
-    for (int i = 0; i < 6; ++i) {
-      const int chunk = threadIdx.x + 256 * i, row = chunk / 24, c8 = chunk - row * 24;
+    const int sb0 = 2 * wn + (NB == 2 ? 0 : 1);
+#pragma unroll
+    for (int i = 0; i < BM * 24 / NT; ++i) {
+      const int chunk = threadIdx.x + NT * i, row = chunk / 24, c8 = chunk - row * 24;
       const int gm = m0 + row < R ? m0 + row : R - 1;
       *reinterpret_cast<uint4*>(Dh + row * AP + c8 * 8) = *reinterpret_cast<const uint4*>(dh + (size_t)gm * H + c8 * 8);
     }
-    WRing<2, H / 16> ring1;
-    gemm_prefetch<2, H / 16>(static_cast<const bf16_t*>(a.w_start_d), a.ks_start_d, 2 * wn, lane, ring1);
+    WRing<1, H / 16> ring1;
+    gemm_prefetch<1, H / 16>(static_cast<const bf16_t*>(a.w_start_d), a.ks_start_d, sb0, lane, ring1);
     __syncthreads();
     PH(1);
-    f32x16_t acc[2];
-    acc_zero<2>(acc);
-    gemm_run<2, H / 16>(static_cast<const bf16_t*>(a.w_start_d), a.ks_start_d, 2 * wn, Dh + (32 * wm + r) * AP + 8 * h, lane, ring1, acc);
-#pragma unroll
-    for (int bn = 0; bn < 2; ++bn)
-#pragma unroll
-      for (int g = 0; g < 4; ++g) {
-        const int n = 32 * (2 * wn + bn) + 8 * g + 4 * h;
-        if (n < HALF)
-          *reinterpret_cast<float4*>(Dt + (32 * wm + r) * ZP + n) = make_float4(acc[bn][4 * g], acc[bn][4 * g + 1], acc[bn][4 * g + 2], acc[bn][4 * g + 3]);
-      }
+    f32x16_t acc[1];
+    acc_zero<1>(acc);
+    gemm_run<1, H / 16>(static_cast<const bf16_t*>(a.w_start_d), a.ks_start_d, sb0, Dh + (32 * wm + r) * AP + 8 * h, lane, ring1, acc);
+#pragma unroll
+    for (int g = 0; g < 4; ++g) {
+      const int n = 32 * sb0 + 8 * g + 4 * h;
+      if (n < HALF)
+        *reinterpret_cast<float4*>(Dt + (32 * wm + r) * ZP + n) = make_float4(acc[0][4 * g], acc[0][4 * g + 1], acc[0][4 * g + 2], acc[0][4 * g + 3]);
+    }
     __syncthreads();
     PH(2);
     float* sL = reinterpret_cast<float*>(smem + B_RED);
-    float* sB = sL + 4 * 64 * 4;
-    float* sW = sB + 4 * 64 * 4;
-    float* sred = sW + 4 * 16;
+    float* sB = sL + NSL * 64 * 4;
+    float* sW = sB + NSL * 64 * 4;
+    float* sred = sW + NSL * 16;
     float extra = 0.f;
     if (blockIdx.x == 0) {
       float sv = 0.f;
-      for (int b = threadIdx.x; b < a.B; b += 256) sv += a.dlogdet[b] * (float)a.len[b];
+      for (int b = threadIdx.x; b < a.B; b += NT) sv += a.dlogdet[b] * (float)a.len[b];
       sv = wave_sum(sv);
       if (lane == 0) sred[wave] = sv;
       __syncthreads();
-      sv = sred[0] + sred[1] + sred[2] + sred[3];
+      sv = ((sred[0] + sred[1]) + (sred[2] + sred[3])) + ((sred[4] + sred[5]) + (sred[6] + sred[7]));
       if (a.pg_partial) extra = sv;
       else {
-        for (int c = threadIdx.x; c < C; c += 256) atomicAdd(a.d_an_logs + c, sv);
+        for (int c = threadIdx.x; c < C; c += NT) atomicAdd(a.d_an_logs + c, sv);
         if (threadIdx.x < 16) atomicAdd(a.d_w_ic + threadIdx.x, (float)G * sv * a.scal[2 + threadIdx.x]);
       }
     }
-    const int g = lane, ph = wave;
+    const int g = lane, ph = wave & 3, rb = 8 * (wave >> 2);
     float accW[16], accL[4] = {0, 0, 0, 0}, accB[4] = {0, 0, 0, 0};
 #pragma unroll
     for (int i = 0; i < 16; ++i) accW[i] = 0.f;
@@ -493,8 +519,7 @@
       for (int i = 0; i < 16; ++i) Wm[i] = a.w_ic[i];
       const float* __restrict__ xp = a.x;
       const float* __restrict__ dip = a.dx_in;
-#pragma unroll
-      for (int rb = 0; rb < BM / 4; rb += 8) {
+      {
         float2 xa[8], xb[8], da[8], db[8];
         float rmv[8];
 #pragma unroll
@@ -544,12 +569,12 @@
     }
     PH(3);
 #pragma unroll
-    for (int k = 0; k < 4; ++k) { sL[(ph * 64 + g) * 4 + k] = accL[k]; sB[(ph * 64 + g) * 4 + k] = accB[k]; }
+    for (int k = 0; k < 4; ++k) { sL[(wave * 64 + g) * 4 + k] = accL[k]; sB[(wave * 64 + g) * 4 + k] = accB[k]; }
 #pragma unroll
     for (int i = 0; i < 16; ++i) accW[i] = wave_sum(accW[i]);
     if (g == 0) {
 #pragma unroll
-      for (int i = 0; i < 16; ++i) sW[ph * 16 + i] = accW[i];
+      for (int i = 0; i < 16; ++i) sW[wave * 16 + i] = accW[i];
     }
     __syncthreads();
     PH(4);
@@ -560,8 +585,8 @@
     }
   } else {
 #pragma unroll
-    for (int k = 0; k < 10; ++k) {
-      const int item = threadIdx.x + 256 * k, row = item / 40, c = 4 * (item - row * 40), gm = m0 + row;
+    for (int k = 0; k < BM * 40 / NT; ++k) {
+      const int item = threadIdx.x + NT * k, row = item / 40, c = 4 * (item - row * 40), gm = m0 + row;
       float4 v = make_float4(0.f, 0.f, 0.f, 0.f);
       if (gm < R) {
         if (a.dz_bct) {
@@ -575,22 +600,26 @@
   }
 
   bf16_t* dout = static_cast<bf16_t*>(a.dout);
-  WRing<3, C / 16> ring2;
-  gemm_prefetch<3, C / 16>(static_cast<const bf16_t*>(a.w_end_d), a.ks_end_d, 3 * wn, lane, ring2);
+  WRing<NB, C / 16> ring2;
+  gemm_prefetch<NB, C / 16>(static_cast<const bf16_t*>(a.w_end_d), a.ks_end_d, nb0, lane, ring2);
   {
-    float4 lr4[5], y14[5];
-    float rmv[5], dldv[5];
-#pragma unroll
-    for (int k = 0; k < 5; ++k) {
-      const int item = threadIdx.x + 256 * k, row = item / 20, c = 4 * (item - row * 20), gm = m0 + row < R ? m0 + row : R - 1;
-      lr4[k] = *reinterpret_cast<const float4*>(a.logs_raw + (size_t)gm * HALF + c);
-      y14[k] = *reinterpret_cast<const float4*>(a.y + (size_t)gm * C + HALF + c);
-      rmv[k] = a.rowmask[gm];
-      dldv[k] = a.dlogdet[a.rowutt[gm]];
-    }
-#pragma unroll
-    for (int k = 0; k < 5; ++k) {
-      const int item = threadIdx.x + 256 * k, row = item / 20, c = 4 * (item - row * 20), gm = m0 + row;
+    constexpr int NCI = (BM * 20 + NT - 1) / NT;
+    float4 lr4[NCI], y14[NCI];
+    float rmv[NCI], dldv[NCI];
+#pragma unroll
+    for (int k = 0; k < NCI; ++k) {
+      const int item = threadIdx.x + NT * k, row = item / 20, c = 4 * (item - row * 20), gm = m0 + row < R ? m0 + row : R - 1;
+      if (item < BM * 20) {
+        lr4[k] = *reinterpret_cast<const float4*>(a.logs_raw + (size_t)gm * HALF + c);
+        y14[k] = *reinterpret_cast<const float4*>(a.y + (size_t)gm * C + HALF + c);
+        rmv[k] = a.rowmask[gm];
+        dldv[k] = a.dlogdet[a.rowutt[gm]];
+      }
+    }
+#pragma unroll
+    for (int k = 0; k < NCI; ++k) {
+      const int item = threadIdx.x + NT * k, row = item / 20, c = 4 * (item - row * 20), gm = m0 + row;
+      if (item >= BM * 20) break;
       uint2 pm = make_uint2(0, 0), pl = make_uint2(0, 0);
       if (gm < R) {
         const float rm = rmv[k];
@@ -624,35 +653,35 @@
   bf16_t* At = Dh;
   const bf16_t* Wsd = static_cast<const bf16_t*>(a.w_skip_d);
   constexpr int KS2 = H / 16, NS = NL * KS2;
-  uint4 ring3[RD][3];
+  uint4 ring3[RD][NB];
   {
-    f32x16_t acc[3];
-    acc_zero<3>(acc);
-    gemm_run<3, C / 16>(static_cast<const bf16_t*>(a.w_end_d), a.ks_end_d, 3 * wn, Dout + (32 * wm + r) * AP + 8 * h, lane, ring2, acc);
+    f32x16_t acc[NB];
+    acc_zero<NB>(acc);
+    gemm_run<NB, C / 16>(static_cast<const bf16_t*>(a.w_end_d), a.ks_end_d, nb0, Dout + (32 * wm + r) * AP + 8 * h, lane, ring2, acc);
     PH(6);
 #pragma unroll
     for (int p = 0; p < RD; ++p)
 #pragma unroll
-      for (int bn = 0; bn < 3; ++bn) ring3[p][bn] = ldfrag(Wsd, (6 * (p / KS2) + 3 * wn + bn) * a.ks_skip_d + p % KS2, lane);
-#pragma unroll
-    for (int bn = 0; bn < 3; ++bn)
+      for (int bn = 0; bn < NB; ++bn) ring3[p][bn] = ldfrag(Wsd, (6 * (p / KS2) + nb0 + bn) * a.ks_skip_d + p % KS2, lane);
+#pragma unroll
+    for (int bn = 0; bn < NB; ++bn)
 #pragma unroll
       for (int g = 0; g < 4; ++g) {
-        const int n = 32 * (3 * wn + bn) + 8 * g + 4 * h;
+        const int n = 32 * (nb0 + bn) + 8 * g + 4 * h;
         const uint2 v = pack4(acc[bn][4 * g] * rm_l, acc[bn][4 * g + 1] * rm_l, acc[bn][4 * g + 2] * rm_l, acc[bn][4 * g + 3] * rm_l);
         *reinterpret_cast<uint2*>(At + (32 * wm + r) * AP + n) = v;
       }
   }
   __syncthreads();
   PH(7);
-  coop_store_rows(static_cast<bf16_t*>(a.dwn_out), H, At, m0, R);
+  coop_store_rows<NT>(static_cast<bf16_t*>(a.dwn_out), H, At, m0, R);
   PH(8);
   bf16_t* via = static_cast<bf16_t*>(a.via_skip);
   const bf16_t* brow = At + (32 * wm + r) * AP + 8 * h;
 #pragma unroll
   for (int l = 0; l < NL; ++l) {
-    f32x16_t acc[3];
-    acc_zero<3>(acc);
+    f32x16_t acc[NB];
+    acc_zero<NB>(acc);
 #pragma unroll
     for (int k0 = 0; k0 < KS2; k0 += 4) {
 #pragma unroll
@@ -660,7 +689,7 @@
         const int st = l * KS2 + kk;
         const bf16x8_t bfm = *reinterpret_cast<const bf16x8_t*>(brow + kk * 16);
 #pragma unroll
-        for (int bn = 0; bn < 3; ++bn) acc[bn] = __builtin_amdgcn_mfma_f32_32x32x16_bf16(asfrag(ring3[st % RD][bn]), bfm, acc[bn], 0, 0, 0);
+        for (int bn = 0; bn < NB; ++bn) acc[bn] = __builtin_amdgcn_mfma_f32_32x32x16_bf16(asfrag(ring3[st % RD][bn]), bfm, acc[bn], 0, 0, 0);
       }
       if (l * KS2 + k0 + RD < NS) {
         __builtin_amdgcn_sched_barrier(0);
@@ -668,28 +697,38 @@
         for (int kk = k0; kk < k0 + 4; ++kk) {
           const int st = l * KS2 + kk, nx = st + RD;
 #pragma unroll
-          for (int bn = 0; bn < 3; ++bn)
-            if (nx < NS) ring3[st % RD][bn] = ldfrag(Wsd, (6 * (nx / KS2) + 3 * wn + bn) * a.ks_skip_d + nx % KS2, lane);
+          for (int bn = 0; bn < NB; ++bn)
+            if (nx < NS) ring3[st % RD][bn] = ldfrag(Wsd, (6 * (nx / KS2) + nb0 + bn) * a.ks_skip_d + nx % KS2, lane);
         }
         __builtin_amdgcn_sched_barrier(0);
       }
     }
     bf16_t* Vst = reinterpret_cast<bf16_t*>(smem + ((l & 1) ? B_DO : B_D));
 #pragma unroll
-    for (int bn = 0; bn < 3; ++bn)
+    for (int bn = 0; bn < NB; ++bn)
 #pragma unroll
       for (int g = 0; g < 4; ++g) {
-        const int n = 32 * (3 * wn + bn) + 8 * g + 4 * h;
+        const int n = 32 * (nb0 + bn) + 8 * g + 4 * h;
         *reinterpret_cast<uint2*>(Vst + (32 * wm + r) * AP + n) = pack4(acc[bn][4 * g], acc[bn][4 * g + 1], acc[bn][4 * g + 2], acc[bn][4 * g + 3]);
       }
     __syncthreads();
-    coop_store_rows(via + l * H, a.ldvs, Vst, m0, R);
+    coop_store_rows<NT>(via + l * H, a.ldvs, Vst, m0, R);
     PH(9 + l);
   }
   if (HEADB && !a.pg_partial) {
     const float* sL = reinterpret_cast<const float*>(smem + B_RED);
-    param_grad_atomics(a, sL, sL + 4 * 64 * 4, sL + 2 * 4 * 64 * 4, wave, lane);
-  }
+    param_grad_atomics(a, sL, sL + NSL * 64 * 4, sL + 2 * NSL * 64 * 4, wave, lane);
+  }
+}
+
+template <bool HEADB, bool TAILB>
+__global__ __launch_bounds__(NT2) WAVES_2 void gt_wn_boundary_bwd_kernel(gt_boundary_bwd_args a)
+{
+  extern __shared__ __attribute__((aligned(16))) unsigned char smem[];
+  const int n_tiles = (a.R + BM - 1) / BM;
+  if ((int)blockIdx.x >= n_tiles) { prefetch_images<NT2>(a.pf_ptr, a.pf_bytes, blockIdx.x - n_tiles, nullptr); return; }
+  if (wave_scalar() < 4) boundary_bwd_wave<HEADB, TAILB, 2>(a, smem);
+  else boundary_bwd_wave<HEADB, TAILB, 1>(a, smem);
 }
 
 __global__ __launch_bounds__(384) void gt_boundary_param_reduce_kernel(const float* __restrict__ pg, int n_wg, float* const* __restrict__ dst)
@@ -713,7 +752,7 @@
 {
   extern __shared__ __attribute__((aligned(16))) unsigned char smem[];
   const int n_tiles = (a.R + BM - 1) / BM;
-  if ((int)blockIdx.x >= n_tiles) { prefetch_images(a.pf_ptr, a.pf_bytes, blockIdx.x - n_tiles, nullptr); return; }
+  if ((int)blockIdx.x >= n_tiles) { prefetch_images<256>(a.pf_ptr, a.pf_bytes, blockIdx.x - n_tiles, nullptr); return; }
   const int lane = threadIdx.x & 63, wave = threadIdx.x >> 6;
   const int r = lane & 31, h = lane >> 5, wm = wave >> 1, wn = wave & 1;
   const int m0 = blockIdx.x * BM, R = a.R;
@@ -759,10 +798,10 @@
     for (int p = 0; p < RD; ++p)
 #pragma unroll
       for (int bn = 0; bn < 3; ++bn) ring[p][bn] = ldfrag(Wskip, (3 * wn + bn) * KK + p, lane);
-    skip_slice<0>(xr[0], As, Wskip, wm, wn, r, h, lane, ring, acc);
-    skip_slice<1>(xr[1], As, Wskip, wm, wn, r, h, lane, ring, acc);
-    skip_slice<2>(xr[2], As, Wskip, wm, wn, r, h, lane, ring, acc);
-    skip_slice<3>(xr[3], As, Wskip, wm, wn, r, h, lane, ring, acc);
+    skip_slice<0, 3, 256>(xr[0], As, Wskip, wm, 3 * wn, r, h, lane, ring, acc);
+    skip_slice<1, 3, 256>(xr[1], As, Wskip, wm, 3 * wn, r, h, lane, ring, acc);
+    skip_slice<2, 3, 256>(xr[2], As, Wskip, wm, 3 * wn, r, h, lane, ring, acc);
+    skip_slice<3, 3, 256>(xr[3], As, Wskip, wm, 3 * wn, r, h, lane, ring, acc);
     WRing<3, H / 16> ring2;
     gemm_prefetch<3, H / 16>(static_cast<const bf16_t*>(a.w_end), a.ks_end, 3 * wn, lane, ring2);
 #pragma unroll
@@ -894,7 +933,7 @@
                   (acc3[bn][4 * g + 2] + b4.z) * rm_l, (acc3[bn][4 * g + 3] + b4.w) * rm_l);
       }
     __syncthreads();
-    coop_store_rows(static_cast<bf16_t*>(a.h_next), H, Hst, m0, R);
+    coop_store_rows<256>(static_cast<bf16_t*>(a.h_next), H, Hst, m0, R);
   }
 }
 
@@ -943,7 +982,7 @@
     attr = true;
   }
   for (int i = 0; i < 16; ++i) if (a.pf_ptr[i] && (!al16(a.pf_ptr[i]) || (a.pf_bytes[i] & 15))) return GT_E_ALIGN;
-  const dim3 grid((a.R + BM - 1) / BM + (a.pf_ptr[0] ? PF_WGS : 0)), block(256);
+  const dim3 grid((a.R + BM - 1) / BM + (a.pf_ptr[0] ? PF_WGS : 0)), block(NT2);
   hipStream_t st = static_cast<hipStream_t>(stream);
   if (tail && head) hipLaunchKernelGGL((gt_wn_boundary_fwd_kernel<true, true>), grid, block, FWD_LDS, st, a);
   else if (tail)    hipLaunchKernelGGL((gt_wn_boundary_fwd_kernel<true, false>), grid, block, FWD_LDS, st, a);
@@ -1034,7 +1073,7 @@
     attr = true;
   }
   for (int i = 0; i < 16; ++i) if (a.pf_ptr[i] && (!al16(a.pf_ptr[i]) || (a.pf_bytes[i] & 15))) return GT_E_ALIGN;
-  const dim3 grid((a.R + BM - 1) / BM + (a.pf_ptr[0] ? PF_WGS : 0)), block(256);
+  const dim3 grid((a.R + BM - 1) / BM + (a.pf_ptr[0] ? PF_WGS : 0)), block(NT2);
   hipStream_t st = static_cast<hipStream_t>(stream);
   if (headb && tailb) hipLaunchKernelGGL((gt_wn_boundary_bwd_kernel<true, true>), grid, block, BWD_LDS, st, a);
   else if (headb)     hipLaunchKernelGGL((gt_wn_boundary_bwd_kernel<true, false>), grid, block, BWD_LDS, st, a);
```

After: 4.528 million mel-frames/s (median of 6 runs). No clear change (+0.6%).
